# bioinfologics/w2rap-contigger

Hardware: NVIDIA B200
Metric: step-2 K=60 graph build Gbases/s (higher is better)
Workload: dtype u64

## Files before the change

### w2rap-contigger_b200/csrc/count_part.cuh

```cuda
#pragma once
#include "kernels.cuh"
#include "shard.cuh"

namespace w2r {

constexpr uint32_t MINI_TILE = 192;
constexpr uint32_t MINI_NU = 8;
constexpr uint32_t MAP_CHUNK = 512;
struct MiniParams {
    uint32_t logP, npass, pass;
    uint32_t* count;
    uint32_t* kcount;
    SkmRec* tmp;
    uint32_t* tpart;
    unsigned long long* tmp_cursor;
    uint64_t tmp_cap;
    int* overflow;
};
__global__ void __launch_bounds__(256, 6) k_minimizer_map(ReadsView r, uint64_t first, uint64_t count, const uint16_t* __restrict__ good, MiniParams mp) {
    __shared__ uint32_t wbuf[8][MINI_TILE];
    __shared__ uint32_t sbuf[8][MINI_TILE];
    uint32_t* wb = wbuf[threadIdx.x >> 5];
    uint32_t* sl = sbuf[threadIdx.x >> 5];
    const uint32_t lane = threadIdx.x & 31u;
// ... 90 lines not shown
__global__ void __launch_bounds__(256) k_scatter_records(ScatterParams sp) {
    const unsigned long long t0 = sp.range[0], t1 = sp.range[1] < sp.tmp_cap ? sp.range[1] : sp.tmp_cap, boff = *sp.batch_off;
    for (unsigned long long i = t0 + (unsigned long long)blockIdx.x * blockDim.x + threadIdx.x; i < t1; i += (unsigned long long)gridDim.x * blockDim.x) {
        const uint32_t b = __ldcs(sp.tpart + i);
        if (b == NIL) continue;
        const ulonglong2* src = reinterpret_cast<const ulonglong2*>(sp.tmp + i);
        const ulonglong2 lo = __ldcs(src), hi = __ldcs(src + 1);
        const unsigned long long pos = boff + sp.base[b] + atomicAdd(sp.cursor + b, 1u);
        if (pos < sp.recs_cap) { ulonglong2* dst = reinterpret_cast<ulonglong2*>(sp.recs + pos); dst[0] = lo; dst[1] = hi; }
        else atomicExch(sp.overflow, 1);
    }
}
__global__ void k_copy_scalar(const unsigned long long* src, unsigned long long* dst) { *dst = *src; }

__global__ void k_next_batch_off(unsigned long long* batch_off, const uint64_t* total) { batch_off[1] = batch_off[0] + *total; }

struct RegionParams {
    CountSlot* region;
    uint32_t logR;
    uint32_t sub_mask, sub_id;
    int* overflow;
};
constexpr uint32_t REGION_MAX_PROBE = 2048;
constexpr uint32_t COUNT_STOP_REGION = 1u << 24;

__device__ __forceinline__ void ld_slot(const CountSlot* q, uint64_t& w0, uint64_t& w1, uint64_t& meta) {
    uint64_t pad;
    asm volatile("ld.global.cg.v4.u64 {%0,%1,%2,%3}, [%4];" : "=l"(w0), "=l"(w1), "=l"(meta), "=l"(pad) : "l"(q));
}

__device__ __forceinline__ void region_insert(const RegionParams& rp, Kmer k, uint32_t ctx, uint64_t h) {
    const uint64_t mask = (1ull << rp.logR) - 1;
    uint64_t s = h >> (64 - rp.logR);
    for (uint32_t probe = 0; probe < REGION_MAX_PROBE; ++probe) {
        CountSlot* q = rp.region + s;
        uint64_t w0, w1, meta;
        ld_slot(q, w0, w1, meta);
        bool hit = false;
        uint32_t have = (uint32_t)(meta >> 32);
        if (w0 == k.w0 && w1 == k.w1) hit = true;
        else if (w0 == EMPTY_W0) {
            U128 old = cas128(q, ~0ull, ~0ull, k.w0, k.w1);
            hit = (old.lo == ~0ull && old.hi == ~0ull) || (old.lo == k.w0 && old.hi == k.w1);
            have = 0;
        }
        if (hit) {
            if ((uint32_t)meta < COUNT_STOP_REGION || w0 == EMPTY_W0) atomicAdd(&q->count, 1u);
            if ((have & ctx) != ctx) atomicOr(&q->ctx, ctx);
            return;
        }
        s = (s + 1) & mask;
    }
    atomicExch(rp.overflow, 1);
}

struct RunView { const uint64_t* part_base; const unsigned long long* slab_off; uint64_t P; const uint32_t* plist; };
__global__ void __launch_bounds__(256) k_count_region(const SkmRec* __restrict__ recs, const uint32_t* __restrict__ sizes, uint32_t b_first, uint32_t gy, RunView rv,
                                                      RegionParams rp) {
    const uint32_t src = blockIdx.y / gy;
    const uint32_t bi = b_first + (blockIdx.y - src * gy);
    const uint32_t b = rv.plist ? rv.plist[bi] : bi;
    const uint64_t n = sizes[(uint64_t)src * rv.P + b];
    const SkmRec* base = recs + rv.slab_off[src] + rv.part_base[(uint64_t)src * rv.P + b];
    const uint32_t lane = threadIdx.x & 31u;
    const uint64_t nw = ((uint64_t)gridDim.x * blockDim.x) >> 5;
    for (uint64_t i = ((uint64_t)blockIdx.x * blockDim.x + threadIdx.x) >> 5; i < n; i += nw) {
        const uint64_t* q = base[i].q;
        if (lane < skm_n(q[3])) {
            Kmer k; uint32_t ctx;
            skm_kmer_at(q, lane, &k, &ctx);
            const uint64_t h = kmer_hash(k);
            if (!rp.sub_mask || (((uint32_t)(h >> 3)) & rp.sub_mask) == rp.sub_id) region_insert(rp, k, ctx, h);
        }
    }
}

constexpr uint32_t SMEM_LOG_SLOTS_MAX = 13;
constexpr uint32_t SMEM_MAX_PROBE = 512;
constexpr uint32_t COUNT_STOP = 1u << 16;
constexpr uint32_t SMEM_MAX_BATCH = 16;
constexpr uint32_t SKM_CHUNK = 1024;
struct SmemCountParams {
    const SkmRec* recs;
    const uint32_t* cursor;
    const uint64_t* part_base;
    const unsigned long long* batch_off;
    uint32_t nbatch;
    uint32_t P;
    uint32_t min_freq;
    unsigned long long* hist;
    ulonglong2* solid_out; unsigned long long* solid_cursor; uint64_t solid_cap; int* solid_overflow;
    DumpRec* dump_out; unsigned long long* dump_cursor;
    uint32_t* failed; unsigned long long* failed_cursor;
    uint32_t log_slots;
    uint32_t chunk;
    const uint32_t* plist; uint32_t nlist;
};

__device__ __forceinline__ uint32_t smem_addr(const void* p) { return (uint32_t)__cvta_generic_to_shared(p); }
__device__ __forceinline__ void mbar_init(uint64_t* bar, uint32_t count) { asm volatile("mbarrier.init.shared::cta.b64 [%0], %1;" ::"r"(smem_addr(bar)), "r"(count)); }
__device__ __forceinline__ void mbar_expect_tx(uint64_t* bar, uint32_t bytes) { asm volatile("mbarrier.expect_tx.relaxed.cta.shared::cta.b64 [%0], %1;" ::"r"(smem_addr(bar)), "r"(bytes) : "memory"); }
__device__ __forceinline__ void mbar_arrive(uint64_t* bar) { asm volatile("{\n\t.reg .b64 st;\n\tmbarrier.arrive.shared::cta.b64 st, [%0];\n\t}" ::"r"(smem_addr(bar)) : "memory"); }
__device__ __forceinline__ void mbar_wait(uint64_t* bar, uint32_t parity) {
    asm volatile(
        "{\n\t.reg .pred p;\n\t"
        "WAIT_%=:\n\t"
        "mbarrier.try_wait.parity.shared::cta.b64 p, [%0], %1;\n\t"
        "@p bra DONE_%=;\n\t"
        "bra WAIT_%=;\n\t"
        "DONE_%=:\n\t}" ::"r"(smem_addr(bar)), "r"(parity) : "memory");
}
__device__ __forceinline__ void bulk_g2s(void* dst, const void* src, uint32_t bytes, uint64_t* bar) {
    asm volatile("cp.async.bulk.shared::cluster.global.mbarrier::complete_tx::bytes [%0], [%1], %2, [%3];" ::"r"(smem_addr(dst)), "l"(src), "r"(bytes), "r"(smem_addr(bar)) : "memory");
}

__device__ __forceinline__ uint32_t smem_slot_hash(Kmer k) {
    uint32_t x = (uint32_t)k.w0 * 0x9e3779b1u + (uint32_t)(k.w0 >> 32) * 0x85ebca77u;
    x ^= x >> 15;
    x += (uint32_t)(k.w1 >> 8) * 0xc2b2ae3du + (uint32_t)(k.w1 >> 40) * 0x27d4eb2fu;
    x ^= x >> 13; x *= 0x165667b1u; x ^= x >> 16;
    return x;
}

__device__ __forceinline__ U128 cas128_shared(void* addr, uint64_t cmp_lo, uint64_t cmp_hi, uint64_t val_lo, uint64_t val_hi) {
    U128 old;
    asm volatile(
        "{\n\t.reg .b128 c, v, o;\n\t"
        "mov.b128 c, {%2, %3};\n\t"
        "mov.b128 v, {%4, %5};\n\t"
        "atom.shared.relaxed.cta.cas.b128 o, [%6], c, v;\n\t"
        "mov.b128 {%0, %1}, o;\n\t}"
        : "=l"(old.lo), "=l"(old.hi)
        : "l"(cmp_lo), "l"(cmp_hi), "l"(val_lo), "l"(val_hi), "r"(smem_addr(addr))
        : "memory");
    return old;
}
__device__ __forceinline__ ulonglong2 lds128_volatile(const void* addr) {
    ulonglong2 v;
    asm volatile("ld.volatile.shared.v2.u64 {%0, %1}, [%2];" : "=l"(v.x), "=l"(v.y) : "r"(smem_addr(addr)) : "memory");
    return v;
}

__global__ void __launch_bounds__(1024, 1) k_count_smem(SmemCountParams sp) {
    extern __shared__ __align__(16) unsigned char smem_raw[];
    const uint32_t SMEM_SLOTS = 1u << sp.log_slots;
    ulonglong2* keys = reinterpret_cast<ulonglong2*>(smem_raw);
    uint32_t* ccs = reinterpret_cast<uint32_t*>(keys + SMEM_SLOTS);
    SkmRec* stage = reinterpret_cast<SkmRec*>(smem_raw + (size_t)20 * SMEM_SLOTS);
    const uint32_t CHUNK = sp.chunk;
    __shared__ __align__(8) uint64_t mbar[2];
    __shared__ unsigned int sh_hist[104];
    __shared__ int sh_fail;
    __shared__ uint32_t sh_tot[2], sh_cnt[2];
    const uint32_t lane = threadIdx.x & 31u, warp = threadIdx.x >> 5, nwarp = blockDim.x >> 5;
    const unsigned le_mask = (2u << lane) - 1u;
    for (int j = threadIdx.x; j < 104; j += blockDim.x) sh_hist[j] = 0;
    if (threadIdx.x == 0) { mbar_init(&mbar[0], 1); mbar_init(&mbar[1], 1); asm volatile("fence.mbarrier_init.release.cluster;" ::: "memory"); }
    __syncthreads();
    const uint32_t n_todo = sp.plist ? sp.nlist : sp.P;
    uint32_t cu_cnt = 0, nx_cnt = 0;
    const SkmRec* cu_src = nullptr; const SkmRec* nx_src = nullptr;
    auto load_desc = [&](uint32_t pi, uint32_t& cnt, const SkmRec*& src) {
        cnt = 0; src = nullptr;
        if (pi < n_todo && lane < sp.nbatch) {
            const uint32_t p = sp.plist ? sp.plist[pi] : pi;
            cnt = sp.cursor[(uint64_t)lane * sp.P + p];
            src = sp.recs + sp.batch_off[lane] + sp.part_base[(uint64_t)lane * sp.P + p];
        }
    };
    auto issue = [&](uint32_t cnt, const SkmRec* src, uint32_t c, uint32_t bf) {
        const uint32_t lo = c * CHUNK, hi = lo + CHUNK;
        uint32_t incl = cnt;
#pragma unroll
        for (int d = 1; d < 32; d <<= 1) { const uint32_t t = __shfl_up_sync(0xffffffffu, incl, d); if ((int)lane >= d) incl += t; }
        const uint32_t acc = incl - cnt, tot = __shfl_sync(0xffffffffu, incl, 31);
        const uint32_t s = acc > lo ? acc : lo, e = acc + cnt < hi ? acc + cnt : hi;
        if (s < e) {
            mbar_expect_tx(&mbar[bf], (e - s) * (uint32_t)sizeof(SkmRec));
            bulk_g2s(stage + (size_t)bf * CHUNK + (s - lo), src + (s - acc), (e - s) * (uint32_t)sizeof(SkmRec), &mbar[bf]);
        }
        __syncwarp();
        if (lane == 0) {
            sh_tot[bf] = tot;
            sh_cnt[bf] = (tot < hi ? tot : hi) - (tot < lo ? tot : lo);
            mbar_arrive(&mbar[bf]);
        }
    };
    uint32_t it = 0;
    if (warp == 0) {
        load_desc(blockIdx.x, cu_cnt, cu_src);
        load_desc(blockIdx.x + gridDim.x, nx_cnt, nx_src);
        if (blockIdx.x < n_todo) issue(cu_cnt, cu_src, 0, 0);
    }
    for (uint32_t pi = blockIdx.x; pi < n_todo; pi += gridDim.x) {
        const uint32_t p = sp.plist ? sp.plist[pi] : pi;
        {
            const ulonglong2 ff = make_ulonglong2(~0ull, ~0ull);
            for (uint32_t j = threadIdx.x; j < SMEM_SLOTS; j += blockDim.x) keys[j] = ff;
            uint4* cw = reinterpret_cast<uint4*>(ccs);
            for (uint32_t j = threadIdx.x; j < SMEM_SLOTS / 4; j += blockDim.x) cw[j] = make_uint4(0, 0, 0, 0);
        }
        if (threadIdx.x == 0) sh_fail = 0;
        __syncthreads();
        auto insert = [&](const Kmer k, const uint32_t ctx) {
            uint32_t s = smem_slot_hash(k) >> (32 - sp.log_slots);
            bool done = false;
            for (uint32_t probe = 0; probe < SMEM_MAX_PROBE && !done; ++probe) {
                ulonglong2 cur = lds128_volatile(keys + s);
                while (cur.x != ~0ull && cur.y == ~0ull) cur = lds128_volatile(keys + s);
                bool mine = cur.x == k.w0 && cur.y == k.w1;
                if (!mine && cur.x == ~0ull) {
                    const U128 old = cas128_shared(keys + s, ~0ull, ~0ull, k.w0, k.w1);
                    mine = (old.lo == ~0ull && old.hi == ~0ull) || (old.lo == k.w0 && old.hi == k.w1);
                }
                if (mine) {
                    const uint32_t old = atomicAdd(ccs + s, 1u);
                    if ((old & 0xffffffu) >= COUNT_STOP) atomicSub(ccs + s, 1u);
                    if ((((old >> 24) & ctx) != ctx)) atomicOr(ccs + s, ctx << 24);
                    done = true;
                } else s = (s + 1u) & (SMEM_SLOTS - 1u);
            }
            if (!done) sh_fail = 1;
        };
        for (uint32_t c = 0;; ++c, ++it) {
            const uint32_t bf = it & 1u;
            mbar_wait(&mbar[bf], (it >> 1) & 1u);
            const uint32_t tot = sh_tot[bf], cnt = sh_cnt[bf];
            const bool more = (uint64_t)(c + 1) * CHUNK < tot;
            if (warp == 0) {
                if (more) issue(cu_cnt, cu_src, c + 1, bf ^ 1u);
                else {
                    if (pi + gridDim.x < n_todo) issue(nx_cnt, nx_src, 0, bf ^ 1u);
                    cu_cnt = nx_cnt; cu_src = nx_src;
                    load_desc(pi + 2 * gridDim.x, nx_cnt, nx_src);
                }
            }
            const SkmRec* st = stage + (size_t)bf * CHUNK;
            const uint32_t share = (cnt + nwarp - 1) / nwarp;
            const uint32_t w_end = (warp + 1) * share < cnt ? (warp + 1) * share : cnt;
            for (uint32_t g0 = warp * share; g0 < w_end; g0 += 32u) {
                const uint32_t gn = w_end - g0 < 32u ? w_end - g0 : 32u;
                const bool have = lane < gn;
                const uint64_t hdr = have ? st[g0 + lane].q[3] : 0ull;
                const uint32_t nr = have ? skm_n(hdr) : 0u;
                uint32_t incl = nr;
#pragma unroll
                for (int d = 1; d < 32; d <<= 1) { const uint32_t t = __shfl_up_sync(0xffffffffu, incl, d); if ((int)lane >= d) incl += t; }
                const uint32_t total = __shfl_sync(0xffffffffu, incl, 31), excl = incl - nr;
                uint32_t before_window = 0;
                for (uint32_t t = 0; t < total; t += 32) {
                    const uint32_t rel = excl - t;
                    const unsigned starts = __reduce_or_sync(0xffffffffu, (nr && rel < 32u) ? 1u << rel : 0u);
                    const uint32_t rr = before_window + (uint32_t)__popc(starts & le_mask) - 1u;
                    const uint32_t r_excl = __shfl_sync(0xffffffffu, excl, rr & 31u);
                    const uint64_t r_hdr = __shfl_sync(0xffffffffu, hdr, rr & 31u);
                    if (t + lane < total) {
                        Kmer k; uint32_t ctx;
                        skm_kmer_at(st[g0 + rr].q, r_hdr, t + lane - r_excl, &k, &ctx);
                        insert(k, ctx);
                    }
                    before_window += (uint32_t)__popc(starts);
                }
            }
            __syncthreads();
            if (!more) { ++it; break; }
        }
        const bool failed = sh_fail != 0;
        if (failed) {
            if (threadIdx.x == 0) sp.failed[atomicAdd(sp.failed_cursor, 1ull)] = p;
        } else {
            for (uint32_t base = 0; base < SMEM_SLOTS; base += blockDim.x) {
                const uint32_t j = base + threadIdx.x;
                const bool in = j < SMEM_SLOTS;
                const ulonglong2 kk = in ? keys[j] : make_ulonglong2(~0ull, ~0ull);
                const bool occ = kk.x != ~0ull;
                const uint32_t cc = in ? ccs[j] : 0u;
                uint32_t c = cc & 0xffffffu; if (c > 255u) c = 255u;
                const uint32_t ctx = cc >> 24;
                const unsigned ones = __ballot_sync(0xffffffffu, occ && c == 1u);
                if (lane == 0 && ones) atomicAdd(&sh_hist[1], (unsigned)__popc(ones));
                if (occ && c != 1u) atomicAdd(&sh_hist[c > 100u ? 100u : c], 1u);
                const bool solid = occ && c >= sp.min_freq;
                const uint64_t pos = warp_append(sp.solid_cursor, solid);
                if (solid) { if (pos < sp.solid_cap) sp.solid_out[pos] = make_ulonglong2(kk.x, kk.y | ctx); else atomicExch(sp.solid_overflow, 1); }
                if (sp.dump_out) {
                    const uint64_t dp = warp_append(sp.dump_cursor, occ);
                    if (occ) sp.dump_out[dp] = DumpRec{kk.x, kk.y, c, ctx, NIL, 0};
                }
            }
        }
        __syncthreads();
    }
    __syncthreads();
    for (int j = threadIdx.x; j <= 100; j += blockDim.x) if (sh_hist[j]) atomicAdd(&sp.hist[j], (unsigned long long)sh_hist[j]);
}

struct ScanParams {
    CountSlot* region;
    uint64_t R;
    uint32_t min_freq;
    unsigned long long* hist;
    ulonglong2* solid_out;
    unsigned long long* solid_cursor;
    uint64_t solid_cap;
    DumpRec* dump_out;
    unsigned long long* dump_cursor;
    const int* overflow;
    int* solid_overflow;
};
__global__ void __launch_bounds__(256) k_scan_region(ScanParams sp) {
    __shared__ unsigned int sh[104];
    for (int j = threadIdx.x; j < 104; j += blockDim.x) sh[j] = 0;
    __syncthreads();
    const bool failed = *sp.overflow != 0;
    uint4* raw = reinterpret_cast<uint4*>(sp.region);
    const uint4 key_empty = make_uint4(0xffffffffu, 0xffffffffu, 0xffffffffu, 0xffffffffu), zero = make_uint4(0, 0, 0, 0);
    for (uint64_t base = (uint64_t)blockIdx.x * blockDim.x; base < sp.R; base += (uint64_t)gridDim.x * blockDim.x) {
        uint64_t i = base + threadIdx.x;
        bool occ = false, solid = false;
        uint32_t c = 0, ctx = 0;
        ulonglong2 k = make_ulonglong2(0, 0);
        if (i < sp.R) {
            k = __ldcg(reinterpret_cast<const ulonglong2*>(sp.region + i));
            if (k.x != EMPTY_W0) {
                occ = true;
                uint2 m = __ldcg(reinterpret_cast<const uint2*>(&sp.region[i].count));
                c = m.x > 255u ? 255u : m.x; ctx = m.y & 0xffu;
                raw[2 * i] = key_empty; raw[2 * i + 1] = zero;
            }
        }
        if (failed) continue;
        uint32_t bin = occ ? (c > 100u ? 100u : c) : 103u;
        unsigned peers = __match_any_sync(0xffffffffu, bin);
        if (occ && (peers & ((1u << lane_id()) - 1u)) == 0) atomicAdd(&sh[bin], (unsigned)__popc(peers));
        solid = occ && c >= sp.min_freq;
        uint64_t pos = warp_append(sp.solid_cursor, solid);
        if (solid) { if (pos < sp.solid_cap) sp.solid_out[pos] = make_ulonglong2(k.x, k.y | ctx); else atomicExch(sp.solid_overflow, 1); }
        if (sp.dump_out) {
            uint64_t dp = warp_append(sp.dump_cursor, occ);
            if (occ) sp.dump_out[dp] = DumpRec{k.x, k.y, c, ctx, NIL, 0};
        }
    }
    __syncthreads();
    if (!failed) {
        for (int j = threadIdx.x; j <= 100; j += blockDim.x) if (sh[j]) atomicAdd(&sp.hist[j], (unsigned long long)sh[j]);
    }
}

}
```

### w2rap-contigger_b200/csrc/extract.cuh

```cuda
#pragma once
#include "kmer.cuh"

namespace w2r {

struct KmerCursor {
    const uint8_t* bases;
    Kmer f, r;
    uint64_t buf;
    uint32_t j, last, prev_first;
    bool live;
    W2R_HD KmerCursor() : bases(nullptr), f{0, 0}, r{0, 0}, buf(0), j(0), last(0), prev_first(0), live(false) {}
    W2R_HD void open(const uint8_t* b, uint32_t good_len) {
        live = good_len > (uint32_t)K;
        if (!live) return;
        bases = b; f = kmer_at(b, 0); r = kmer_rc(f); last = good_len - K; j = 0; prev_first = 0; buf = 0;
    }
    W2R_HD bool next(Kmer* canon, uint32_t* ctx) {
        if (!live) return false;
        uint32_t nxt = 0, c = 0;
        if ((j & 31u) == 0) buf = bases32_at(bases, (uint64_t)j + K);
        if (j < last) { nxt = (uint32_t)buf & 3u; c |= 1u << nxt; }
        buf >>= 2;
        if (j > 0) c |= 16u << prev_first;
        const bool rev = kmer_less(r, f);
        *canon = Kmer{rev ? r.w0 : f.w0, rev ? r.w1 : f.w1};
        *ctx = rev ? ctx_rc(c) : c;
        if (j == last) live = false;
        else { prev_first = kmer_first(f); f = kmer_succ(f, nxt); r = kmer_pred(r, 3u - nxt); ++j; }
        return true;
    }
};

template <class Emit>
W2R_HD void extract_read_kmers(const uint8_t* bases, uint32_t good_len, Emit& emit) {
    KmerCursor cur;
    cur.open(bases, good_len);
    Kmer k; uint32_t ctx;
    while (cur.next(&k, &ctx)) emit(k, ctx);
}

constexpr uint32_t SKM_MAX = 32;
struct alignas(16) SkmRec { uint64_t q[4]; };
W2R_HD uint32_t skm_n(uint64_t hdr) { return (uint32_t)((hdr >> 56) & 31u) + 1u; }
W2R_HD SkmRec skm_build(const uint8_t* bases, uint32_t j_first, uint32_t n, uint32_t last) {
    const uint32_t hp = j_first > 0 ? 1u : 0u, hs = j_first + n - 1u < last ? 1u : 0u;
    const uint64_t p0 = (uint64_t)j_first - hp;
    const uint32_t bits = 2u * (n + (uint32_t)K - 1u + hp + hs);
    const uintptr_t addr = (uintptr_t)bases + (uintptr_t)(p0 >> 2);
    const uint64_t* w = (const uint64_t*)(addr & ~(uintptr_t)7);
    const uint32_t sh = (uint32_t)(addr & 7u) * 8u + (uint32_t)(p0 & 3u) * 2u;
    const uint64_t a = w[0], b = w[1], c = w[2], d = w[3];
    SkmRec r;
    r.q[0] = sh ? (a >> sh) | (b << (64u - sh)) : a;
    r.q[1] = sh ? (b >> sh) | (c << (64u - sh)) : b;
    r.q[2] = sh ? (c >> sh) | (d << (64u - sh)) : c;
    if (bits < 128u) { r.q[1] &= (1ull << (bits - 64u)) - 1ull; r.q[2] = 0; }
    else if (bits < 192u) r.q[2] = bits > 128u ? r.q[2] & ((1ull << (bits - 128u)) - 1ull) : 0ull;
    r.q[3] = ((uint64_t)(n - 1u) << 56) | ((uint64_t)hp << 61) | ((uint64_t)hs << 62);
    return r;
}
W2R_HD void skm_kmer_at(const uint64_t* q, uint64_t hdr , uint32_t j, Kmer* canon, uint32_t* ctx) {
    const uint32_t n = skm_n(hdr), hp = (uint32_t)(hdr >> 61) & 1u, hs = (uint32_t)(hdr >> 62) & 1u;
    const uint32_t b = 2u * (hp + j), wo = b >> 6, sh = b & 63u;
    const uint64_t A = q[wo], B = q[wo + 1], C = wo ? 0ull : q[2];
    const uint64_t lo = sh ? (A >> sh) | (B << (64u - sh)) : A;
    const uint64_t hi = sh ? (B >> sh) | (C << (64u - sh)) : B;
    const Kmer f{rev2(lo), rev2(hi) & ~0xffull};
    const Kmer rc{(~hi << 8) | (~lo >> 56), ~lo << 8};
    uint32_t c = 0;
    if (j + 1u < n || hs) c |= 1u << ((uint32_t)(hi >> 56) & 3u);
    if (j > 0u || hp) c |= 16u << (sh ? (uint32_t)(A >> (sh - 2u)) & 3u : (uint32_t)(q[wo - 1] >> 62));
    const bool rev = kmer_less(rc, f);
    *canon = Kmer{rev ? rc.w0 : f.w0, rev ? rc.w1 : f.w1};
    *ctx = rev ? ctx_rc(c) : c;
}
W2R_HD void skm_kmer_at(const uint64_t* q, uint32_t j, Kmer* canon, uint32_t* ctx) { skm_kmer_at(q, q[3], j, canon, ctx); }

constexpr int MINI_M = 15;
constexpr int MINI_W = K - MINI_M + 1;
W2R_HD uint32_t mmer_hash_of(uint32_t v) {
    const uint32_t rc = rev2_32(~v) >> (32 - 2 * MINI_M);
    uint32_t c = v < rc ? v : rc;
    c ^= c >> 16; c *= 0x85ebca6bu; c ^= c >> 13; c *= 0xc2b2ae35u; c ^= c >> 16;
    return c;
}
W2R_HD uint32_t mmer_hash_at(const uint8_t* bases, uint64_t pos) { return mmer_hash_of(bases16_at(bases, pos) & ((1u << (2 * MINI_M)) - 1u)); }
W2R_HD uint32_t mini_mix(uint32_t wmin) {
    uint32_t x = wmin * 0x9e3779b1u;
    x ^= x >> 15; x *= 0x2c1b3c6du; x ^= x >> 13;
    return x;
}
W2R_HD uint32_t mini_part(uint32_t mixed, uint32_t logP) { return logP ? mixed >> (32u - logP) : 0u; }
W2R_HD uint32_t kmer_minimizer_hash_words(Kmer k) {
    const uint64_t lo = rev2(k.w0), hi = rev2(k.w1);
    uint32_t m = 0xffffffffu;
    for (int t = 0; t < MINI_W; ++t) {
        const int bit = 2 * t;
        const uint64_t w = bit == 0 ? lo : (bit < 64 ? (lo >> bit) | (hi << (64 - bit)) : hi >> (bit - 64));
        const uint32_t h = mmer_hash_of((uint32_t)w & ((1u << (2 * MINI_M)) - 1u));
        if (h < m) m = h;
    }
    return m;
}
W2R_HD uint32_t kmer_minimizer_hash(const uint8_t* bases, uint64_t j) {
    uint32_t m = 0xffffffffu;
    for (int t = 0; t < MINI_W; ++t) { const uint32_t h = mmer_hash_at(bases, j + t); if (h < m) m = h; }
    return m;
}

}
```

### w2rap-contigger_b200/csrc/kernels.cuh

```cuda
#pragma once
#include "extract.cuh"
#include "kmer.cuh"
#include "path.cuh"
#include "pqvec.cuh"
#include "rt.cuh"
#include "unipath.cuh"

namespace w2r {

struct ReadsView {
    uint64_t n;
    const uint8_t* bases;
    const uint64_t* base_off;
    const uint32_t* len;
    const uint8_t* quals;
    const uint64_t* qual_off;
};

struct U128 { uint64_t lo, hi; };

__device__ __forceinline__ U128 cas128(void* addr, uint64_t cmp_lo, uint64_t cmp_hi, uint64_t val_lo, uint64_t val_hi) {
    U128 old;
    asm volatile(
        "{\n\t.reg .b128 c, v, o;\n\t"
        "mov.b128 c, {%2, %3};\n\t"
        "mov.b128 v, {%4, %5};\n\t"
        "atom.global.relaxed.gpu.cas.b128 o, [%6], c, v;\n\t"
        "mov.b128 {%0, %1}, o;\n\t}"
        : "=l"(old.lo), "=l"(old.hi)
        : "l"(cmp_lo), "l"(cmp_hi), "l"(val_lo), "l"(val_hi), "l"(addr)
        : "memory");
    return old;
}

__device__ __forceinline__ unsigned lane_id() { return threadIdx.x & 31u; }

__device__ __forceinline__ uint64_t warp_append(unsigned long long* cursor, bool want) {
    unsigned active = __activemask();
    unsigned m = __ballot_sync(active, want);
    if (!want) return 0;
    int leader = __ffs(m) - 1;
    unsigned long long base = 0;
    if ((int)lane_id() == leader) base = atomicAdd(cursor, (unsigned long long)__popc(m));
    base = __shfl_sync(m, base, leader);
    return base + __popc(m & ((1u << lane_id()) - 1u));
}
__device__ __forceinline__ void warp_add(unsigned long long* counter, unsigned long long v) {
    unsigned active = __activemask();
    for (int d = 16; d > 0; d >>= 1) v += __shfl_down_sync(active, v, d);
    if (lane_id() == 0 && v) atomicAdd(counter, v);
}


__global__ void k_init_count_table(CountSlot* tab, uint64_t T) {
    const uint4 key = make_uint4(0xffffffffu, 0xffffffffu, 0xffffffffu, 0xffffffffu), zero = make_uint4(0, 0, 0, 0);
    uint4* p = reinterpret_cast<uint4*>(tab);
    for (uint64_t i = (uint64_t)blockIdx.x * blockDim.x + threadIdx.x; i < 2 * T; i += (uint64_t)gridDim.x * blockDim.x) p[i] = (i & 1) ? zero : key;
}

__global__ void k_good_len(ReadsView r, uint64_t first, uint64_t count, uint32_t min_qual, uint16_t* __restrict__ good, unsigned long long* __restrict__ n_inst,
                           int* __restrict__ bad) {
    const uint64_t end = first + count;
    for (uint64_t base = first + (uint64_t)blockIdx.x * blockDim.x; base < end; base += (uint64_t)gridDim.x * blockDim.x) {
        uint64_t i = base + threadIdx.x;
        unsigned long long mine = 0;
        if (i < end) {
            uint32_t nq = 0;
            uint32_t gl = pq_good_length(r.quals + r.qual_off[i], r.quals + r.qual_off[i + 1], min_qual, &nq);
            if (nq != r.len[i]) atomicExch(bad, 1);
            if (gl > r.len[i]) gl = r.len[i];
            good[i] = (uint16_t)gl;
            if (gl > (uint32_t)K) mine = gl - K + 1;
        }
        unsigned active = __activemask();
        for (int d = 16; d > 0; d >>= 1) mine += __shfl_down_sync(active, mine, d);
        if (lane_id() == 0 && mine) atomicAdd(n_inst, mine);
    }
}

struct DumpRec { uint64_t w0, w1; uint32_t count, ctx, edge, off; };
__global__ void k_dump_solid(SolidTable st, DumpRec* __restrict__ out, unsigned long long* cursor) {
    const uint64_t T = st.size();
    for (uint64_t base = (uint64_t)blockIdx.x * blockDim.x; base < T; base += (uint64_t)gridDim.x * blockDim.x) {
        uint64_t i = base + threadIdx.x;
        bool want = i < T && st.slots[i].w0 != EMPTY_W0;
        uint64_t pos = warp_append(cursor, want);
        if (want) { const SolidSlot& s = st.slots[i]; out[pos] = DumpRec{s.w0, s.w1, 0, s.ctx & 0xffu, s.edge, s.off}; }
    }
}

__global__ void k_insert_solid(const ulonglong2* __restrict__ recs, uint64_t n, SolidTable st, uint32_t* __restrict__ bloom, uint32_t bloom_W, uint32_t slice_words) {
    for (uint64_t i = (uint64_t)blockIdx.x * blockDim.x + threadIdx.x; i < n; i += (uint64_t)gridDim.x * blockDim.x) {
        ulonglong2 rec = __ldcs(recs + i);
        Kmer k{rec.x, rec.y & ~0xffull};
        uint32_t ctx = (uint32_t)rec.y & 0xffu;
        if (bloom) { const uint32_t bh = bloom_hash(k); atomicOr(bloom + pd_bloom_word(bloom_W, slice_words, bh), bloom_mask(bh)); }
        uint64_t h = st.home(k);
        for (;;) {
            SolidSlot* p = st.slots + h;
            U128 old = cas128(p, ~0ull, ~0ull, k.w0, k.w1);
            if (old.lo == ~0ull && old.hi == ~0ull) { p->ctx = ctx; p->edge = NIL; p->off = 0; p->pad = 0; break; }
            h = st.next(h);
        }
    }
}
__global__ void k_insert_entries(const SolidSlot* __restrict__ recs, uint64_t n, SolidTable st, uint32_t* __restrict__ bloom, uint32_t bloom_W, uint32_t slice_words) {
    for (uint64_t i = (uint64_t)blockIdx.x * blockDim.x + threadIdx.x; i < n; i += (uint64_t)gridDim.x * blockDim.x) {
        const SolidSlot e = recs[i];
        if (bloom) { const uint32_t bh = bloom_hash(Kmer{e.w0, e.w1}); atomicOr(bloom + pd_bloom_word(bloom_W, slice_words, bh), bloom_mask(bh)); }
        uint64_t h = st.home(Kmer{e.w0, e.w1});
        for (;;) {
            SolidSlot* p = st.slots + h;
            U128 old = cas128(p, ~0ull, ~0ull, e.w0, e.w1);
            if (old.lo == ~0ull && old.hi == ~0ull) { p->ctx = e.ctx; p->edge = e.edge; p->off = e.off; p->pad = 0; break; }
            h = st.next(h);
        }
    }
}

__global__ void k_adjacency(SolidTable st) {
    const uint64_t T = st.size();
    for (uint64_t i = (uint64_t)blockIdx.x * blockDim.x + threadIdx.x; i < T; i += (uint64_t)gridDim.x * blockDim.x) {
        SolidSlot* s = st.slots + i;
        if (s->w0 == EMPTY_W0 || slot_is_ghost(*s)) continue;
        uint32_t c = s->ctx & 0xffu;
        uint32_t c2 = pruned_context(st, Kmer{s->w0, s->w1}, c);
        if (c2 != c) s->ctx = c2;
    }
}

__global__ void k_links(SolidTable st, uint32_t* __restrict__ next0, int* __restrict__ missing) {
    const uint64_t nn = 2 * st.size();
    for (uint64_t x = (uint64_t)blockIdx.x * blockDim.x + threadIdx.x; x < nn; x += (uint64_t)gridDim.x * blockDim.x) {
        int miss = 0;
        next0[x] = unipath_succ_link(st, (uint32_t)x, &miss);
        if (miss) atomicExch(missing, 1);
    }
}
__global__ void k_rank_init(const uint32_t* __restrict__ next0, uint64_t nn, RankState* __restrict__ A) {
    for (uint64_t x = (uint64_t)blockIdx.x * blockDim.x + threadIdx.x; x < nn; x += (uint64_t)gridDim.x * blockDim.x) A[x] = rank_init_node(next0, (uint32_t)x);
}
__global__ void k_rank_init_list(const uint32_t* __restrict__ list, uint64_t n, const uint32_t* __restrict__ next0, RankState* __restrict__ A) {
    for (uint64_t i = (uint64_t)blockIdx.x * blockDim.x + threadIdx.x; i < n; i += (uint64_t)gridDim.x * blockDim.x) { uint32_t x = list[i]; A[x] = rank_init_node(next0, x); }
}
__global__ void k_rank_step(const uint32_t* __restrict__ list, uint64_t n, const RankState* __restrict__ A, RankState* __restrict__ B, unsigned long long* __restrict__ unresolved) {
    for (uint64_t base = (uint64_t)blockIdx.x * blockDim.x; base < n; base += (uint64_t)gridDim.x * blockDim.x) {
        uint64_t i = base + threadIdx.x;
        bool un = false;
        if (i < n) {
            uint32_t x = list ? list[i] : (uint32_t)i;
            B[x] = rank_step_node(A, x, &un);
        }
        unsigned m = __ballot_sync(__activemask(), un);
        if (lane_id() == 0 && m) atomicAdd(unresolved, (unsigned long long)__popc(m));
    }
}
__global__ void k_rank_step_inplace(const uint32_t* __restrict__ list, uint64_t n, unsigned long long* S, unsigned long long* __restrict__ unresolved) {
    for (uint64_t base = (uint64_t)blockIdx.x * blockDim.x; base < n; base += (uint64_t)gridDim.x * blockDim.x) {
        uint64_t i = base + threadIdx.x;
        bool un = false;
        if (i < n) {
            uint32_t x = list[i];
            unsigned long long a = __ldcg(S + x);
            uint32_t ax = (uint32_t)a, ay = (uint32_t)(a >> 32);
            if (!(ay & RANK_RESOLVED)) {
                unsigned long long b = __ldcg(S + ax);
                uint32_t bx = (uint32_t)b, by = (uint32_t)(b >> 32);
                ay = (ay + (by & ~RANK_RESOLVED)) | (by & RANK_RESOLVED);
                __stcg(S + x, (unsigned long long)bx | ((unsigned long long)ay << 32));
                un = !(ay & RANK_RESOLVED);
            }
        }
        unsigned m = __ballot_sync(__activemask(), un);
        if (lane_id() == 0 && m) atomicAdd(unresolved, (unsigned long long)__popc(m));
    }
}
__global__ void k_count_splitters(const uint32_t* __restrict__ next0, const uint8_t* __restrict__ ghead, uint64_t nn, unsigned long long* __restrict__ count) {
    for (uint64_t base = (uint64_t)blockIdx.x * blockDim.x; base < nn; base += (uint64_t)gridDim.x * blockDim.x) {
        uint64_t x = base + threadIdx.x;
        const unsigned m = __ballot_sync(__activemask(), x < nn && node_is_splitter(next0, ghead, (uint32_t)x));
        if (lane_id() == 0 && m) atomicAdd(count, (unsigned long long)__popc(m));
    }
}
__global__ void k_list_splitters(const uint32_t* __restrict__ next0, const uint8_t* __restrict__ ghead, uint64_t nn, uint32_t* __restrict__ list, uint64_t list_cap,
                                 unsigned long long* cursor) {
    for (uint64_t base = (uint64_t)blockIdx.x * blockDim.x; base < nn; base += (uint64_t)gridDim.x * blockDim.x) {
        uint64_t x = base + threadIdx.x;
        bool sp = x < nn && node_is_splitter(next0, ghead, (uint32_t)x);
        uint64_t pos = warp_append(cursor, sp);
        if (sp && pos < list_cap) list[pos] = (uint32_t)x;
    }
}
__global__ void k_splitter_walk(const uint32_t* __restrict__ next0, const uint32_t* __restrict__ list, uint64_t n, RankState* __restrict__ label, RankState* __restrict__ S) {
    for (uint64_t i = (uint64_t)blockIdx.x * blockDim.x + threadIdx.x; i < n; i += (uint64_t)gridDim.x * blockDim.x) splitter_walk(next0, list[i], label, S);
}
__global__ void k_splitter_finish(const uint32_t* __restrict__ next0, uint64_t nn, RankState* __restrict__ label_then_rank, const RankState* __restrict__ S,
                                  unsigned long long* __restrict__ unresolved) {
    for (uint64_t base = (uint64_t)blockIdx.x * blockDim.x; base < nn; base += (uint64_t)gridDim.x * blockDim.x) {
        uint64_t x = base + threadIdx.x;
        bool un = false;
        if (x < nn) { RankState r = splitter_finish_node(next0, label_then_rank, S, (uint32_t)x); label_then_rank[x] = r; un = !(r.y & RANK_RESOLVED); }
        unsigned m = __ballot_sync(__activemask(), un);
        if (lane_id() == 0 && m) atomicAdd(unresolved, (unsigned long long)__popc(m));
    }
}
__global__ void k_copy_list(const uint32_t* __restrict__ list, uint64_t n, const RankState* __restrict__ src, RankState* __restrict__ dst) {
    for (uint64_t i = (uint64_t)blockIdx.x * blockDim.x + threadIdx.x; i < n; i += (uint64_t)gridDim.x * blockDim.x) dst[list[i]] = src[list[i]];
}
__global__ void k_collect_unresolved(const RankState* __restrict__ A, uint64_t nn, uint32_t* __restrict__ list, unsigned long long* cursor) {
    for (uint64_t base = (uint64_t)blockIdx.x * blockDim.x; base < nn; base += (uint64_t)gridDim.x * blockDim.x) {
        uint64_t x = base + threadIdx.x;
        bool want = x < nn && !(A[x].y & RANK_RESOLVED);
        uint64_t pos = warp_append(cursor, want);
        if (want) list[pos] = (uint32_t)x;
    }
}
__global__ void k_cycle_init(const uint32_t* __restrict__ list, uint64_t n, const uint32_t* __restrict__ next0, RankState* __restrict__ A) {
    for (uint64_t i = (uint64_t)blockIdx.x * blockDim.x + threadIdx.x; i < n; i += (uint64_t)gridDim.x * blockDim.x) {
        uint32_t x = list[i];
        A[x] = RankState{next0[x], x >> 1};
    }
}
__global__ void k_cycle_step(const uint32_t* __restrict__ list, uint64_t n, SolidTable st, const RankState* __restrict__ A, RankState* __restrict__ B, int* __restrict__ changed) {
    for (uint64_t i = (uint64_t)blockIdx.x * blockDim.x + threadIdx.x; i < n; i += (uint64_t)gridDim.x * blockDim.x) {
        uint32_t x = list[i];
        bool ch;
        B[x] = cycle_step_node(st, A, x, &ch);
        if (ch) *changed = 1;
    }
}
__global__ void k_cycle_cut(const uint32_t* __restrict__ list, uint64_t n, const RankState* __restrict__ A, uint32_t* __restrict__ next0) {
    for (uint64_t i = (uint64_t)blockIdx.x * blockDim.x + threadIdx.x; i < n; i += (uint64_t)gridDim.x * blockDim.x) {
        cycle_cut_node(A, next0, list[i]);
    }
}
__global__ void k_strand_decide(SolidTable st, const RankState* __restrict__ R, uint8_t* __restrict__ keep, int* __restrict__ too_long) {
    const uint64_t nn = 2 * st.size();
    for (uint64_t xi = (uint64_t)blockIdx.x * blockDim.x + threadIdx.x; xi < nn; xi += (uint64_t)gridDim.x * blockDim.x) {
        if (strand_decide_node(st, R, (uint32_t)xi, keep)) atomicExch(too_long, 1);
    }
}
__global__ void k_collect_heads(SolidTable st, const RankState* __restrict__ R, const uint8_t* __restrict__ keep, uint32_t* __restrict__ h_node,
                                uint64_t* __restrict__ h_w0, uint64_t* __restrict__ h_w1, uint32_t* __restrict__ h_n, unsigned long long* cursor, uint64_t cap) {
    const uint64_t nn = 2 * st.size();
    for (uint64_t base = (uint64_t)blockIdx.x * blockDim.x; base < nn; base += (uint64_t)gridDim.x * blockDim.x) {
        uint64_t xi = base + threadIdx.x;
        bool want = false;
        uint32_t x = (uint32_t)xi;
        if (xi < nn) want = head_is_kept(st, R, keep, x);
        uint64_t pos = warp_append(cursor, want);
        if (want && pos < cap) {
            Kmer k = node_kmer(st, x);
            h_node[pos] = x; h_w0[pos] = k.w0; h_w1[pos] = k.w1; h_n[pos] = (R[x].y & ~RANK_RESOLVED) + 1u;
        }
    }
}
__global__ void k_assign_edges(const uint32_t* __restrict__ perm, uint64_t E, const uint32_t* __restrict__ h_node, const uint32_t* __restrict__ h_n,
                               uint32_t* __restrict__ edge_of_head, uint32_t* __restrict__ edge_len, uint32_t* __restrict__ edge_nbytes) {
    for (uint64_t i = (uint64_t)blockIdx.x * blockDim.x + threadIdx.x; i < E; i += (uint64_t)gridDim.x * blockDim.x) {
        uint32_t j = perm[i];
        edge_of_head[h_node[j]] = (uint32_t)i;
        uint32_t len = h_n[j] + K - 1;
        edge_len[i] = len;
        edge_nbytes[i] = (len + 3) / 4;
    }
}
struct OrBase {
    uint8_t* bases;
    __device__ __forceinline__ void operator()(uint64_t byte_off, uint64_t pos, uint32_t b) const {
        uint64_t addr = byte_off + (pos >> 2);
        atomicOr(reinterpret_cast<uint32_t*>(bases + (addr & ~3ull)), b << (8 * (uint32_t)(addr & 3ull) + 2 * (uint32_t)(pos & 3ull)));
    }
};
__global__ void k_emit_edges(SolidTable st, const RankState* __restrict__ R, const uint32_t* __restrict__ edge_of_head, const uint64_t* __restrict__ edge_off,
                             uint8_t* __restrict__ edge_bases) {
    const uint64_t nn = 2 * st.size();
    OrBase put{edge_bases};
    for (uint64_t xi = (uint64_t)blockIdx.x * blockDim.x + threadIdx.x; xi < nn; xi += (uint64_t)gridDim.x * blockDim.x) emit_node(st, R, edge_of_head, edge_off, (uint32_t)xi, put);
}

__global__ void k_copy_to_host(const uint8_t* __restrict__ src, uint8_t* __restrict__ dst, size_t bytes) {
    const size_t n16 = bytes / 16;
    const uint4* s4 = reinterpret_cast<const uint4*>(src);
    uint4* d4 = reinterpret_cast<uint4*>(dst);
    for (size_t i = (size_t)blockIdx.x * blockDim.x + threadIdx.x; i < n16; i += (size_t)gridDim.x * blockDim.x) d4[i] = s4[i];
    if (blockIdx.x == 0 && threadIdx.x < (bytes & 15)) dst[n16 * 16 + threadIdx.x] = src[n16 * 16 + threadIdx.x];
}

__global__ void k_edge_ends(const uint8_t* __restrict__ edge_bases, const uint64_t* __restrict__ edge_off, const uint32_t* __restrict__ edge_len, uint64_t E,
                            uint64_t* __restrict__ kh, uint64_t* __restrict__ k0, uint64_t* __restrict__ k1, uint8_t* __restrict__ is_pal) {
    for (uint64_t idx = (uint64_t)blockIdx.x * blockDim.x + threadIdx.x; idx < 4 * E; idx += (uint64_t)gridDim.x * blockDim.x) {
        uint64_t e = idx >> 2;
        uint32_t w = (uint32_t)idx & 3u;
        bool pal; EndKey key;
        edge_end_key(edge_bases + edge_off[e], edge_len[e], w, &pal, &key);
        if (w == 0) is_pal[e] = pal ? 1 : 0;
        kh[idx] = key.h; k0[idx] = key.k0; k1[idx] = key.k1;
    }
}
__global__ void k_vertex_flags(const uint32_t* __restrict__ perm, uint64_t n4, const uint64_t* __restrict__ kh, const uint64_t* __restrict__ k0,
                               const uint64_t* __restrict__ k1, uint32_t* __restrict__ flag) {
    for (uint64_t i = (uint64_t)blockIdx.x * blockDim.x + threadIdx.x; i < n4; i += (uint64_t)gridDim.x * blockDim.x) {
        uint32_t j = perm[i];
        bool valid = !(kh[j] == ~0ull && k0[j] == ~0ull && k1[j] == ~0ull);
        uint32_t fl = 0;
        if (valid) {
            if (i == 0) fl = 1;
            else { uint32_t q = perm[i - 1]; fl = (kh[q] != kh[j] || k0[q] != k0[j] || k1[q] != k1[j]) ? 1u : 0u; }
        }
        flag[i] = fl;
    }
}
__global__ void k_hash_order_check(const uint32_t* __restrict__ perm, uint64_t n4, const uint64_t* __restrict__ kh, const uint64_t* __restrict__ k0,
                                   const uint64_t* __restrict__ k1, unsigned long long* __restrict__ collisions) {
    for (uint64_t i = (uint64_t)blockIdx.x * blockDim.x + threadIdx.x + 1; i < n4; i += (uint64_t)gridDim.x * blockDim.x) {
        const uint32_t j = perm[i], q = perm[i - 1];
        if (kh[q] == kh[j] && (k0[q] != k0[j] || k1[q] != k1[j])) atomicAdd(collisions, 1ull);
    }
}
__global__ void k_scatter_vids(const uint32_t* __restrict__ perm, uint64_t n4, const uint32_t* __restrict__ flag, const uint32_t* __restrict__ excl,
                               const uint64_t* __restrict__ kh, const uint64_t* __restrict__ k0, const uint64_t* __restrict__ k1, int32_t* __restrict__ edge_vertices) {
    for (uint64_t i = (uint64_t)blockIdx.x * blockDim.x + threadIdx.x; i < n4; i += (uint64_t)gridDim.x * blockDim.x) {
        uint32_t j = perm[i];
        bool valid = !(kh[j] == ~0ull && k0[j] == ~0ull && k1[j] == ~0ull);
        edge_vertices[j] = valid ? (int32_t)(excl[i] + flag[i]) - 1 : -1;
    }
}
__global__ void k_pal_widths(const uint8_t* __restrict__ is_pal, uint64_t E, uint32_t* __restrict__ width) {
    for (uint64_t i = (uint64_t)blockIdx.x * blockDim.x + threadIdx.x; i < E; i += (uint64_t)gridDim.x * blockDim.x) width[i] = is_pal[i] ? 1u : 2u;
}
__global__ void k_hbv_edges(uint64_t E, const uint8_t* __restrict__ is_pal, const uint32_t* __restrict__ xl, const int32_t* __restrict__ edge_vertices,
                            int32_t* __restrict__ fwd_xlat, int32_t* __restrict__ rev_xlat, uint32_t* __restrict__ hcanon, int32_t* __restrict__ hleft, int32_t* __restrict__ hright,
                            int32_t* __restrict__ involution) {
    for (uint64_t i = (uint64_t)blockIdx.x * blockDim.x + threadIdx.x; i < E; i += (uint64_t)gridDim.x * blockDim.x) {
        uint32_t f = xl[i];
        fwd_xlat[i] = (int32_t)f;
        hcanon[f] = (uint32_t)(i << 1); hleft[f] = edge_vertices[4 * i]; hright[f] = edge_vertices[4 * i + 1];
        if (is_pal[i]) { rev_xlat[i] = (int32_t)f; involution[f] = (int32_t)f; }
        else {
            rev_xlat[i] = (int32_t)f + 1; hcanon[f + 1] = (uint32_t)(i << 1) | 1u; hleft[f + 1] = edge_vertices[4 * i + 2]; hright[f + 1] = edge_vertices[4 * i + 3];
            involution[f] = (int32_t)f + 1; involution[f + 1] = (int32_t)f;
        }
    }
}
__global__ void k_adj_fill(uint64_t nh, const int32_t* __restrict__ hleft, const int32_t* __restrict__ hright, int32_t* __restrict__ from_e, int32_t* __restrict__ to_e,
                           uint32_t* __restrict__ from_cnt, uint32_t* __restrict__ to_cnt, int* __restrict__ bad) {
    for (uint64_t he = (uint64_t)blockIdx.x * blockDim.x + threadIdx.x; he < nh; he += (uint64_t)gridDim.x * blockDim.x) {
        int32_t l = hleft[he], r = hright[he];
        uint32_t a = atomicAdd(&from_cnt[l], 1u);
        if (a < 4) from_e[4 * (int64_t)l + a] = (int32_t)he; else atomicExch(bad, 1);
        uint32_t b = atomicAdd(&to_cnt[r], 1u);
        if (b < 4) to_e[4 * (int64_t)r + b] = (int32_t)he; else atomicExch(bad, 1);
    }
}
__global__ void k_adj_sort(uint64_t nv, const int32_t* __restrict__ hleft, const int32_t* __restrict__ hright, int32_t* __restrict__ from_e, int32_t* __restrict__ to_e,
                           const uint32_t* __restrict__ from_cnt, const uint32_t* __restrict__ to_cnt, uint8_t* __restrict__ from_n, uint8_t* __restrict__ to_n) {
    for (uint64_t v = (uint64_t)blockIdx.x * blockDim.x + threadIdx.x; v < nv; v += (uint64_t)gridDim.x * blockDim.x) {
        for (int dir = 0; dir < 2; ++dir) {
            int32_t* lst = (dir ? to_e : from_e) + 4 * v;
            const int32_t* nb = dir ? hleft : hright;
            uint32_t n = dir ? to_cnt[v] : from_cnt[v];
            if (n > 4) n = 4;
            for (uint32_t i = 1; i < n; ++i) {
                int32_t e = lst[i]; int32_t ke = nb[e];
                int j = (int)i - 1;
                while (j >= 0 && (nb[lst[j]] > ke || (nb[lst[j]] == ke && lst[j] > e))) { lst[j + 1] = lst[j]; --j; }
                lst[j + 1] = e;
            }
            (dir ? to_n : from_n)[v] = (uint8_t)n;
        }
    }
}

struct alignas(8) PathMeta { uint32_t x, y; };
constexpr int PATH_GAP_BATCH = 4;
template <int MIN_CTAS>
__global__ void __launch_bounds__(128, MIN_CTAS) k_path_reads(ReadsView r, GraphView g, const uint32_t* __restrict__ list, uint64_t n_rows,
                                                    int32_t* __restrict__ stage, uint32_t cap, uint32_t left_cap, int32_t* __restrict__ out_offset,
                                                    PathMeta* __restrict__ out_meta, uint32_t apply_fixpaths) {
    struct Slot { PathState st; uint32_t pad[(sizeof(PathState) / 4) % 2 == 0 ? 1 : 2]; };
    __shared__ Slot slots[128];
    PathState& ps = slots[threadIdx.x].st;
    const uint32_t lane = lane_id();
    const uint64_t stride = (uint64_t)gridDim.x * blockDim.x;
    for (uint64_t row0 = (uint64_t)blockIdx.x * blockDim.x + (threadIdx.x & ~31u); row0 < n_rows; row0 += stride) {
        const uint64_t row = row0 + lane;
        const bool live = row < n_rows;
        const uint64_t i = live ? (list ? list[row] : row) : 0;
        PathWalker w(ps);
        w.init(g, r.bases + r.base_off[i], live ? r.len[i] : 0u, stage + (live ? row : 0) * cap, cap, left_cap);
        bool need = false, run = true, have_gap = false;
        uint32_t from = 0, found_p = 0;
        const SolidSlot* found_slot = nullptr;
        for (;;) {
            if (run) {
                if (have_gap) w.gap_found(found_p, found_slot);
                need = w.scan();
                from = ps.itr + 1u;
                run = false; have_gap = false;
            }
            unsigned m = __ballot_sync(0xffffffffu, need);
            if (!m) break;
            uint32_t cand = 0;
            while (m) {
                int src[PATH_GAP_BATCH];
                uint32_t word[PATH_GAP_BATCH], bits[PATH_GAP_BATCH];
                int n = 0;
#pragma unroll
                for (int q = 0; q < PATH_GAP_BATCH; ++q) { src[q] = m ? __ffs((int)m) - 1 : -1; if (m) { m &= m - 1; ++n; } }
#pragma unroll
                for (int q = 0; q < PATH_GAP_BATCH; ++q) {
                    word[q] = 0; bits[q] = 1;
                    if (q < n) {
                        const uint8_t* b = reinterpret_cast<const uint8_t*>(__shfl_sync(0xffffffffu, reinterpret_cast<unsigned long long>(ps.bases), src[q]));
                        const uint32_t p = __shfl_sync(0xffffffffu, from, src[q]) + lane, nk = __shfl_sync(0xffffffffu, ps.nk, src[q]);
                        if (p < nk) {
                            Kmer f, rc;
                            kmer_pair_at(b, p, &f, &rc);
                            const uint32_t hh = bloom_hash(kmer_less(rc, f) ? rc : f);
                            if (g.dict.bloom) { word[q] = __ldg(g.dict.bloom + pd_bloom_word(g.dict.W, g.dict.slice_words, hh)); bits[q] = bloom_mask(hh); }
                            else { word[q] = 1; bits[q] = 1; }
                        }
                    }
                }
#pragma unroll
                for (int q = 0; q < PATH_GAP_BATCH; ++q) {
                    if (q < n) {
                        const unsigned mm = __ballot_sync(0xffffffffu, (word[q] & bits[q]) == bits[q]);
                        if ((int)lane == src[q]) cand = mm;
                    }
                }
// ... 93 lines not shown
```

### w2rap-contigger_b200/csrc/pipeline.cu

```cuda
#include <algorithm>
#include <cmath>
#include <chrono>
#include <cstdarg>
#include <exception>
#include <map>
#include <mutex>
#include <thread>
#include <unordered_map>

#include <cuda.h>

#include "../../include/w2rap_step2.h"
#include "device_reads.cuh"
#include "count_part.cuh"
#include "kernels.cuh"
#include "shardgraph_kernels.cuh"
#include "nccl_dl.h"
#include "prims.cuh"
#include "slab_freelist.h"
#include "places.cuh"

namespace w2r {

static double now_ms() { return std::chrono::duration<double, std::milli>(std::chrono::steady_clock::now().time_since_epoch()).count(); }
// ... 131 lines not shown
                    CUmemAccessDesc acc = {};
                    acc.location = prop.location; acc.flags = CU_MEM_ACCESS_FLAGS_PROT_READWRITE;
                    if (v.Map(base + mapped, take, 0, h, 0) == CUDA_SUCCESS && v.SetAccess(base + mapped, take, &acc, 1) == CUDA_SUCCESS) {
                        v.Release(h);
                        fl.add_free(mapped, take);
                        mapped += take;
                        return true;
                    }
                    v.Release(h);
                    return false;
                }
            }
            cudaMemPool_t pool;
            if (attempt == 0 && cudaDeviceGetDefaultMemPool(&pool, device) == cudaSuccess) { cudaDeviceSynchronize(); cudaMemPoolTrimTo(pool, 0); } else break;
        }
        return false;
    }
    void* acquire(size_t bytes) {
        bytes = (bytes + ALIGN - 1) / ALIGN * ALIGN;
        size_t off = fl.take(bytes);
        if (off == SlabFreeList::NONE) {
            if (!grow(bytes - fl.free_tail(mapped))) return nullptr;
            off = fl.take(bytes);
            if (off == SlabFreeList::NONE) return nullptr;
        }
        return (void*)(base + off);
    }
    void release(void* p) { fl.give_back((size_t)((CUdeviceptr)p - base)); }
};
struct SlabLease {
    DeviceSlab* slab = nullptr;
    explicit SlabLease(int device) {
        DeviceSlab& s = DeviceSlab::get(device);
        if (s.lease.try_lock()) { if (s.init(device)) slab = &s; else s.lease.unlock(); }
    }
    ~SlabLease() {
        if (!slab) return;
        if (std::uncaught_exceptions() > 0) cudaDeviceSynchronize();
        slab->lease.unlock();
    }
    SlabLease(const SlabLease&) = delete;
    SlabLease& operator=(const SlabLease&) = delete;
};

template <class T>
struct SBuf {
    T* p = nullptr;
    size_t n = 0;
    cudaStream_t s = nullptr;
    DeviceSlab* slab = nullptr;
    SBuf() {}
    SBuf(Ctx& c, size_t n_) { alloc(c, n_); }
    SBuf(const SBuf&) = delete;
    SBuf& operator=(const SBuf&) = delete;
    SBuf(SBuf&& o) noexcept : p(o.p), n(o.n), s(o.s), slab(o.slab) { o.p = nullptr; o.n = 0; o.slab = nullptr; }
    SBuf& operator=(SBuf&& o) noexcept { if (this != &o) { release(); p = o.p; n = o.n; s = o.s; slab = o.slab; o.p = nullptr; o.n = 0; o.slab = nullptr; } return *this; }
    ~SBuf() { release(); }
    void alloc(Ctx& c, size_t n_) {
        release();
        s = c.stream; n = n_;
        if (!n) return;
        const double t0 = now_ms();
        const size_t bytes = n * sizeof(T);
        DeviceSlab* sl = (DeviceSlab*)c.slab;
        if (sl && bytes >= DeviceSlab::MIN_BYTES) { p = (T*)sl->acquire(bytes); if (p) slab = sl; }
        cudaError_t e = cudaSuccess;
        if (!p) e = cudaMallocAsync((void**)&p, bytes, s);
        const double dt = now_ms() - t0;
        g_alloc_host_ms += dt;
        if (dt > 20.0 && getenv("W2RAP_TRACE")) fprintf(stderr, "[w2rap] device allocation of %.2f GB took %.1f ms on the host\n", bytes / 1e9, dt);
        W2R_CUDA(e);
    }
    void release() {
        if (p) {
            const double t0 = now_ms();
            if (slab) slab->release(p); else cudaFreeAsync(p, s);
            g_alloc_host_ms += now_ms() - t0;
        }
        p = nullptr; n = 0; slab = nullptr;
    }
    size_t bytes() const { return n * sizeof(T); }
    void zero() { if (n) W2R_CUDA(cudaMemsetAsync(p, 0, bytes(), s)); }
    void fill_ff() { if (n) W2R_CUDA(cudaMemsetAsync(p, 0xff, bytes(), s)); }
};

static size_t device_budget(const Ctx& c) {
    size_t fr = 0, tot = 0;
    W2R_CUDA(cudaMemGetInfo(&fr, &tot));
    cudaMemPool_t pool;
    if (cudaDeviceGetDefaultMemPool(&pool, c.device) == cudaSuccess) {
        uint64_t reserved = 0, used = 0;
        cudaMemPoolGetAttribute(pool, cudaMemPoolAttrReservedMemCurrent, &reserved);
        cudaMemPoolGetAttribute(pool, cudaMemPoolAttrUsedMemCurrent, &used);
        if (reserved > used) fr += (size_t)(reserved - used);
    }
    if (c.slab) fr += ((const DeviceSlab*)c.slab)->idle_bytes();
    return fr;
}

struct StageTimer {
    Ctx& c;
    cudaEvent_t ev[2];
    explicit StageTimer(Ctx& c_) : c(c_) { cudaEventCreate(&ev[0]); cudaEventCreate(&ev[1]); }
    ~StageTimer() { cudaEventDestroy(ev[0]); cudaEventDestroy(ev[1]); }
    void start() { cudaEventRecord(ev[0], c.stream); }
    float stop() { cudaEventRecord(ev[1], c.stream); cudaEventSynchronize(ev[1]); float ms = 0; cudaEventElapsedTime(&ms, ev[0], ev[1]); return ms; }
};

struct KernelTimers {
    struct Span { int idx; cudaEvent_t a, b; };
    std::vector<Span> spans;
    cudaStream_t s = nullptr;
    void begin(int idx) { Span sp{idx, nullptr, nullptr}; cudaEventCreate(&sp.a); cudaEventCreate(&sp.b); cudaEventRecord(sp.a, s); spans.push_back(sp); }
    void end() { cudaEventRecord(spans.back().b, s); }
    void resolve(float* kernel_ms) {
        for (Span& sp : spans) {
            float ms = 0;
            if (cudaEventSynchronize(sp.b) == cudaSuccess && cudaEventElapsedTime(&ms, sp.a, sp.b) == cudaSuccess) kernel_ms[sp.idx] += ms; else cudaGetLastError();
            cudaEventDestroy(sp.a); cudaEventDestroy(sp.b);
        }
        spans.clear();
    }
    ~KernelTimers() { for (Span& sp : spans) { cudaEventDestroy(sp.a); cudaEventDestroy(sp.b); } }
};
#define W2R_TIMED(idx, ...) do { kt_.begin(idx); __VA_ARGS__; kt_.end(); } while (0)

static void say(const Ctx& c, const char* fmt, ...) {
    if (!c.verbose) return;
    va_list ap; va_start(ap, fmt); vprintf(fmt, ap); va_end(ap); printf("\n"); fflush(stdout);
}

struct Pipeline {
    Ctx c;
    const DeviceReads& dr;
    const w2rap_params& prm;
    w2rap_graph* out;
    GraphOwner* owner;
    std::vector<DumpRec> dump_host;
    KernelTimers kt_;

    double trace_t0 = 0;
    void trace_mark(const char* what) {
        static const bool on = getenv("W2RAP_TRACE") != nullptr;
        if (!on) return;
        cudaStreamSynchronize(c.stream);
        const double t = now_ms();
        if (trace_t0 && rank == 0) fprintf(stderr, "[w2rap] %-28s %8.1f ms   (allocator so far %.1f ms)\n", what, t - trace_t0, g_alloc_host_ms);
        trace_t0 = t;
    }

    SBuf<uint16_t> good;
    SBuf<SolidSlot> solid_slots;
    SolidTable st{nullptr, 0};
    uint64_t E = 0, nv = 0, nh = 0;
    SBuf<uint8_t> edge_bases; SBuf<uint64_t> edge_off; SBuf<uint32_t> edge_len;
    SBuf<int32_t> edge_vertices, fwd_xlat, rev_xlat, involution, hleft, hright, from_e, to_e;
    SBuf<uint32_t> hcanon;
    SBuf<uint8_t> from_n, to_n;
    uint64_t edge_bytes = 0;
    int world = 1, rank = 0;
    ncclComm_t comm = nullptr;

    Pipeline(const DeviceReads& dr_, const w2rap_params& p_, w2rap_graph* out_, GraphOwner* ow) : dr(dr_), prm(p_), out(out_), owner(ow) {}

    unsigned grid(uint64_t n, unsigned block, unsigned per_sm = 16) const { return grid_for(c, n, block, per_sm); }

    void set_l2_window(void* base, size_t bytes) {
        cudaStreamAttrValue attr;
        memset(&attr, 0, sizeof attr);
        attr.accessPolicyWindow.base_ptr = base;
        attr.accessPolicyWindow.num_bytes = bytes;
        attr.accessPolicyWindow.hitRatio = 1.0f;
        attr.accessPolicyWindow.hitProp = bytes ? cudaAccessPropertyPersisting : cudaAccessPropertyNormal;
        attr.accessPolicyWindow.missProp = bytes ? cudaAccessPropertyStreaming : cudaAccessPropertyNormal;
        if (cudaStreamSetAttribute(c.stream, cudaStreamAttributeAccessPolicyWindow, &attr) != cudaSuccess) cudaGetLastError();
    }

    void nccl_check(ncclResult_t r, const char* what) {
        if (r != ncclSuccess) W2R_FAIL(W2RAP_ERR_CUDA, "NCCL %s failed: %s", what, NcclApi::get().GetErrorString ? NcclApi::get().GetErrorString(r) : "?");
    }
    void allreduce_u64(std::vector<unsigned long long>& v, ncclRedOp_t op) {
        if (world == 1) return;
        SBuf<unsigned long long> d(c, v.size());
        W2R_CUDA(cudaMemcpyAsync(d.p, v.data(), v.size() * 8, cudaMemcpyHostToDevice, c.stream));
        nccl_check(NcclApi::get().AllReduce(d.p, d.p, v.size(), ncclUint64, op, comm, c.stream), "all-reduce");
        W2R_CUDA(cudaMemcpyAsync(v.data(), d.p, v.size() * 8, cudaMemcpyDeviceToHost, c.stream));
        W2R_CUDA(cudaStreamSynchronize(c.stream));
    }
    void alltoall_slabs(const void* send, void* recv, size_t slab_bytes) {
        NcclApi& n = NcclApi::get();
        nccl_check(n.GroupStart(), "group start");
        for (int peer = 0; peer < world; ++peer) {
            if (peer == rank) continue;
            nccl_check(n.Send((const char*)send + (size_t)peer * slab_bytes, slab_bytes, ncclUint8, peer, comm, c.stream), "send");
            nccl_check(n.Recv((char*)recv + (size_t)peer * slab_bytes, slab_bytes, ncclUint8, peer, comm, c.stream), "recv");
        }
        nccl_check(n.GroupEnd(), "group end");
        W2R_CUDA(cudaMemcpyAsync((char*)recv + (size_t)rank * slab_bytes, (const char*)send + (size_t)rank * slab_bytes, slab_bytes, cudaMemcpyDeviceToDevice, c.stream));
    }

    void alltoall_v(const void* send, const std::vector<size_t>& soff, const std::vector<size_t>& scnt, void* recv, const std::vector<size_t>& roff,
                    const std::vector<size_t>& rcnt) {
        NcclApi& n = NcclApi::get();
        nccl_check(n.GroupStart(), "group start");
        for (int peer = 0; peer < world; ++peer) {
            if (peer == rank) continue;
            if (scnt[peer]) nccl_check(n.Send((const char*)send + soff[peer], scnt[peer], ncclUint8, peer, comm, c.stream), "send");
            if (rcnt[peer]) nccl_check(n.Recv((char*)recv + roff[peer], rcnt[peer], ncclUint8, peer, comm, c.stream), "recv");
        }
        nccl_check(n.GroupEnd(), "group end");
        if (scnt[rank]) W2R_CUDA(cudaMemcpyAsync((char*)recv + roff[rank], (const char*)send + soff[rank], scnt[rank], cudaMemcpyDeviceToDevice, c.stream));
    }

    struct Batch { uint64_t first, count; cudaEvent_t ready; };
    struct CountPlan {
        uint32_t logP = 0, npass = 1, nmap = 1, nslab = 1;
        uint64_t P = 1, Pown = 1;
        uint64_t n_inst = 0, n_inst_local = 0;
    };
    struct CountBufs {
        SBuf<SkmRec> recs, xrecs;
        SBuf<SkmRec> tmp; SBuf<uint32_t> tpart;
        SBuf<unsigned long long> tmp_cursor, tmp_range;
        SBuf<uint32_t> part_count, part_kcount, cursor;
        SBuf<uint64_t> part_base, batch_total, batch_ktotal;
        SBuf<unsigned long long> batch_off;
        SBuf<uint32_t> xcount, xkcount;
        SBuf<uint64_t> xbase, xtot, xktot;
        SBuf<unsigned long long> xoff;
    };
    SBuf<unsigned long long> cs_scal;
    SBuf<int> cs_flags;
    SBuf<unsigned long long> cs_hist;
    SBuf<CountSlot> cs_region;
    SBuf<DumpRec> cs_dump;
    SBuf<ulonglong2> cs_solid; uint64_t cs_solid_cap = 0;
    uint64_t cs_R = 0; uint32_t cs_logR = 0;
    bool good_done = false;
    float map_ms = 0, reduce_ms = 0, xchg_ms = 0;
    uint32_t n_groups = 0;
    uint64_t xchg_bytes = 0, xchg_count_bytes = 0, n_records = 0;

    void run_good_len(const Batch& bt) {
        if (bt.ready) W2R_CUDA(cudaStreamWaitEvent(c.stream, bt.ready, 0));
        if (bt.count) W2R_TIMED(W2RAP_KT_GOOD_LEN, W2R_LAUNCH(c, k_good_len, grid(bt.count, 128), 128, 0, dr.view(), bt.first, bt.count, prm.min_qual, good.p, cs_scal.p, cs_flags.p));
    }

    static unsigned map_ctas() {
        static const unsigned n = getenv("W2RAP_MAP_CTAS") ? (unsigned)atoi(getenv("W2RAP_MAP_CTAS")) : 6u;
        return n;
    }
    uint64_t map_chunk_warps(uint64_t count) const { return std::min<uint64_t>(count, (uint64_t)grid(count * 32, 256, map_ctas()) * 8); }

    bool map_records(const CountPlan& pl, CountBufs& cb, const std::vector<Batch>& batches, uint32_t pass, uint64_t* need) {
        const ReadsView rv = dr.view();
        const uint64_t P = pl.P;
        cb.cursor.zero(); cb.part_count.zero(); cb.part_kcount.zero();
        W2R_CUDA(cudaMemsetAsync(cb.batch_off.p, 0, sizeof(unsigned long long), c.stream));
        std::vector<Batch> mb = batches;
        if (world > 1) {
            if (!good_done) for (const Batch& bt : batches) run_good_len(bt);
            good_done = true;
            mb.assign(1, Batch{0, dr.n, nullptr});
        }
        std::vector<cudaEvent_t> ev(2 * pl.nmap, nullptr);
        struct EvGuard { std::vector<cudaEvent_t>& v; ~EvGuard() { for (cudaEvent_t e : v) if (e) cudaEventDestroy(e); } } evg{ev};
        W2R_CUDA(cudaMemsetAsync(cb.tmp_cursor.p, 0, 8, c.stream));
        W2R_CUDA(cudaMemsetAsync(cb.tpart.p, 0xff, cb.tpart.bytes(), c.stream));
        for (uint32_t bi = 0; bi < pl.nmap; ++bi) {
            const Batch& bt = mb[bi];
            MiniParams mp{pl.logP, pl.npass, pass, cb.part_count.p + bi * P, cb.part_kcount.p + bi * P, cb.tmp.p, cb.tpart.p, cb.tmp_cursor.p, cb.tmp.n, cs_flags.p + 1};
            ScatterParams sp{cb.tmp.p, cb.tpart.p, cb.tmp_range.p + bi, cb.part_base.p + bi * P, cb.cursor.p + bi * P, cb.recs.p, cb.batch_off.p + bi, cb.recs.n, cb.tmp.n, cs_flags.p + 1};
            if (!good_done) run_good_len(bt);
            W2R_CUDA(cudaEventCreate(&ev[2 * bi])); W2R_CUDA(cudaEventCreate(&ev[2 * bi + 1]));
            W2R_CUDA(cudaEventRecord(ev[2 * bi], c.stream));
            W2R_LAUNCH(c, k_copy_scalar, 1, 1, 0, (const unsigned long long*)cb.tmp_cursor.p, cb.tmp_range.p + bi);
            if (bt.count && pl.n_inst_local) W2R_TIMED(W2RAP_KT_MAP, W2R_LAUNCH(c, k_minimizer_map, grid(bt.count * 32, 256, map_ctas()), 256, 0, rv, bt.first, bt.count, good.p, mp));
            W2R_LAUNCH(c, k_copy_scalar, 1, 1, 0, (const unsigned long long*)cb.tmp_cursor.p, cb.tmp_range.p + bi + 1);
            exclusive_scan<uint32_t, uint64_t>(c, cb.part_count.p + bi * P, P, cb.part_base.p + bi * P, cb.batch_total.p + bi);
            W2R_LAUNCH(c, k_next_batch_off, 1, 1, 0, cb.batch_off.p + bi, cb.batch_total.p + bi);
            if (bt.count && pl.n_inst_local) { W2R_TIMED(W2RAP_KT_SCATTER, W2R_LAUNCH(c, k_scatter_records, (unsigned)(c.sm_count * 8), 256, 0, sp)); c.count_launches++; }
            W2R_CUDA(cudaEventRecord(ev[2 * bi + 1], c.stream));
        }
        good_done = true;
        unsigned long long total = 0, staged = 0;
        W2R_CUDA(cudaMemcpyAsync(&total, cb.batch_off.p + pl.nmap, 8, cudaMemcpyDeviceToHost, c.stream));
        W2R_CUDA(cudaMemcpyAsync(&staged, cb.tmp_cursor.p, 8, cudaMemcpyDeviceToHost, c.stream));
        W2R_CUDA(cudaStreamSynchronize(c.stream));
        for (uint32_t bi = 0; bi < pl.nmap; ++bi) { float ms = 0; cudaEventElapsedTime(&ms, ev[2 * bi], ev[2 * bi + 1]); map_ms += ms; }
        if (d2h_scalar(c, cs_flags.p)) W2R_FAIL(W2RAP_ERR_BAD_ARG, "a read's quality vector does not have one quality per base");
        n_records += total;
        *need = std::max(total, staged);
        std::vector<unsigned long long> of = {(unsigned long long)d2h_scalar(c, cs_flags.p + 1)};
        allreduce_u64(of, ncclMax);
        if (of[0]) { W2R_CUDA(cudaMemsetAsync(cs_flags.p + 1, 0, sizeof(int), c.stream)); return false; }
        return true;
    }

    void exchange_records(const CountPlan& pl, CountBufs& cb) {
        EventTimer kt(c.stream);
        kt.start();
        const uint64_t Pown = pl.Pown;
        alltoall_slabs(cb.part_count.p, cb.xcount.p, Pown * sizeof(uint32_t));
        alltoall_slabs(cb.part_kcount.p, cb.xkcount.p, Pown * sizeof(uint32_t));
        W2R_CUDA(cudaMemsetAsync(cb.xoff.p, 0, sizeof(unsigned long long), c.stream));
        for (int sidx = 0; sidx < world; ++sidx) {
// ... 169 lines not shown
        cs_dump.alloc(c, prm.dump_kmers == 2 ? pl.n_inst : 0);
        W2R_LAUNCH(c, k_init_count_table, grid(4 * cs_R, 256), 256, 0, cs_region.p, 2 * cs_R);
        cudaStream_t s2 = nullptr;
        W2R_CUDA(cudaStreamCreateWithFlags(&s2, cudaStreamNonBlocking));
        struct StreamGuard { cudaStream_t s; ~StreamGuard() { if (s) { cudaStreamSynchronize(s); cudaStreamDestroy(s); } } } s2_guard{s2};
        cudaEvent_t ev_fork, ev_join;
        cudaEventCreateWithFlags(&ev_fork, cudaEventDisableTiming); cudaEventCreateWithFlags(&ev_join, cudaEventDisableTiming);
        struct EventGuard { cudaEvent_t a, b; ~EventGuard() { cudaEventDestroy(a); cudaEventDestroy(b); } } ev_guard{ev_fork, ev_join};

        std::vector<unsigned long long> rk = {dr.n_kreads};
        allreduce_u64(rk, ncclSum);
        double rec_per_inst = pl.n_inst ? std::min(1.0, 1.15 * ((double)rk[0] + 0.074 * (double)pl.n_inst) / (double)pl.n_inst) : 1.0;
        uint64_t need_exact = 0;
        pl.npass = prm.force_passes ? prm.force_passes : 1u;
        for (int attempt = 0;; ++attempt) {
            if (attempt > 12) W2R_FAIL(W2RAP_ERR_INTERNAL, "k-mer partitioning did not converge");
            const uint64_t P = pl.P, Pown = pl.Pown;
            const size_t local_recs = std::max<uint64_t>(need_exact + need_exact / 64, (uint64_t)((double)pl.n_inst_local * rec_per_inst / pl.npass * (pl.npass > 1 ? 1.25 : 1.0))) + 1024;
            const size_t solid_est = (size_t)((double)pl.n_inst / world / pl.npass / std::max<uint32_t>(1, prm.min_freq) * 1.3) * sizeof(ulonglong2);
            const size_t rec_bytes = (local_recs * 2 + local_recs / 8 + (world > 1 ? (size_t)((double)pl.n_inst * rec_per_inst / world / pl.npass * 1.25) : 0)) * (sizeof(SkmRec) + 4);
            std::vector<unsigned long long> too_big = {(rec_bytes + solid_est + cs_dump.bytes() + (64u << 20) > budget) ? 1ull : 0ull};
            allreduce_u64(too_big, ncclMax);
            if (too_big[0] && !prm.force_passes) {
                if (pl.npass >= 4096) W2R_FAIL(W2RAP_ERR_OOM, "not enough device memory for the k-mer records even in 4096 passes");
                pl.npass *= 2; --attempt; continue;
            }
            CountBufs cb;
            uint64_t chunk_warps = 0;
            if (world > 1) chunk_warps = map_chunk_warps(dr.n);
            else for (const Batch& bt : batches) chunk_warps += map_chunk_warps(bt.count);
            const size_t stage_recs = local_recs + local_recs / 8 + chunk_warps * MAP_CHUNK;
            cb.tmp_cursor.alloc(c, 1); cb.tmp_range.alloc(c, pl.nmap + 1);
            cb.part_count.alloc(c, pl.nmap * P); cb.part_kcount.alloc(c, pl.nmap * P); cb.cursor.alloc(c, pl.nmap * P);
            cb.part_base.alloc(c, pl.nmap * P); cb.batch_total.alloc(c, pl.nmap); cb.batch_ktotal.alloc(c, pl.nmap);
            cb.batch_off.alloc(c, pl.nmap + 1);
            if (world > 1) {
                cb.xcount.alloc(c, world * Pown); cb.xkcount.alloc(c, world * Pown); cb.xbase.alloc(c, world * Pown);
                cb.xtot.alloc(c, world); cb.xktot.alloc(c, world); cb.xoff.alloc(c, world + 1);
            }
            bool retry = false;
            W2R_CUDA(cudaMemsetAsync(cs_scal.p + 1, 0, 16, c.stream));
            cs_hist.zero();
            n_groups = 0;
            uint64_t solid_used = 0;
            for (uint32_t pass = 0; pass < pl.npass && !retry; ++pass) {
                uint64_t need = 0;
                cb.recs.alloc(c, local_recs);
                cb.tmp.alloc(c, stage_recs); cb.tpart.alloc(c, stage_recs);
                trace_mark("count: buffers");
                const bool mapped = map_records(pl, cb, batches, pass, &need);
                trace_mark("count: map+scatter");
                cb.tmp.release(); cb.tpart.release();
                if (!mapped) {
                    std::vector<unsigned long long> nd = {need};
                    allreduce_u64(nd, ncclMax);
                    need_exact = std::max<uint64_t>(need_exact, nd[0]);
                    retry = true; break;
                }
                if (world > 1) { exchange_records(pl, cb); cb.recs.release(); }
                trace_mark("count: exchange");
                const uint32_t* xcur = world > 1 ? cb.xcount.p : cb.part_count.p;
                const uint32_t* xkcur = world > 1 ? cb.xkcount.p : cb.part_kcount.p;
                const SkmRec* xrecs = world > 1 ? cb.xrecs.p : cb.recs.p;
                RunView runs = world > 1 ? RunView{cb.xbase.p, cb.xoff.p, Pown, nullptr} : RunView{cb.part_base.p, cb.batch_off.p, Pown, nullptr};
                {
                    SBuf<uint64_t> ktot(c, pl.nslab), kscan(c, Pown);
                    for (uint32_t sidx = 0; sidx < pl.nslab; ++sidx) exclusive_scan<uint32_t, uint64_t>(c, xkcur + (uint64_t)sidx * Pown, Pown, kscan.p, ktot.p + sidx);
                    std::vector<uint64_t> kt_h(pl.nslab);
                    W2R_CUDA(cudaMemcpyAsync(kt_h.data(), ktot.p, pl.nslab * 8, cudaMemcpyDeviceToHost, c.stream));
                    W2R_CUDA(cudaStreamSynchronize(c.stream));
                    uint64_t owned = 0;
                    for (uint64_t v : kt_h) owned += v;
                    const uint64_t want = solid_used + owned / std::max<uint32_t>(1, prm.min_freq) + 1024;
                    if (want > cs_solid_cap) {
                        SBuf<ulonglong2> bigger(c, want + want / 4);
                        if (solid_used) W2R_CUDA(cudaMemcpyAsync(bigger.p, cs_solid.p, solid_used * sizeof(ulonglong2), cudaMemcpyDeviceToDevice, c.stream));
                        cs_solid = std::move(bigger);
                        cs_solid_cap = cs_solid.n;
                    }
                }
                trace_mark("count: solid staging");
                reduce_records(pl, xrecs, xcur, xkcur, runs, s2, ev_fork, ev_join);
                trace_mark("count: reduce");
                solid_used = d2h_scalar(c, cs_scal.p + 1);
                if (world > 1) cb.xrecs.release();
            }
            if (retry) continue;
            if (d2h_scalar(c, cs_flags.p + 2)) W2R_FAIL(W2RAP_ERR_INTERNAL, "solid staging buffer overflow");
            break;
        }
        {
            std::vector<unsigned long long> exact = {(unsigned long long)d2h_scalar(c, cs_scal.p)};
            allreduce_u64(exact, ncclSum);
            out->n_kmer_instances = exact[0];
            say(c, "%llu k-mer instances in quality-floored reads", exact[0]);
        }
        out->timings.count_kernel_ms = map_ms;
        out->timings.region_ms = reduce_ms;
        out->timings.exchange_ms = xchg_ms;
        out->timings.count_passes = n_groups;
        std::vector<unsigned long long> hh(104);
        W2R_CUDA(cudaMemcpyAsync(hh.data(), cs_hist.p, 104 * 8, cudaMemcpyDeviceToHost, c.stream));
        unsigned long long cursors[2];
        W2R_CUDA(cudaMemcpyAsync(cursors, cs_scal.p + 1, 16, cudaMemcpyDeviceToHost, c.stream));
        W2R_CUDA(cudaStreamSynchronize(c.stream));
        allreduce_u64(hh, ncclSum);
        uint64_t n_distinct = 0;
        for (int i = 1; i <= 100; ++i) { out->hist[i] = hh[i]; n_distinct += hh[i]; }
        const uint64_t n_solid_local = cursors[0];
        if (prm.dump_kmers == 2 && cursors[1]) {
            dump_host.resize(cursors[1]);
            W2R_CUDA(cudaMemcpyAsync(dump_host.data(), cs_dump.p, cursors[1] * sizeof(DumpRec), cudaMemcpyDeviceToHost, c.stream));
            W2R_CUDA(cudaStreamSynchronize(c.stream));
        }
        cs_region.release(); cs_dump.release();
        build_dictionary(n_solid_local, n_distinct);
    }

    void alloc_path_filter(uint64_t n_solid) {
        path_slice_words = 0;
        path_bloom.release();
        if (n_solid < 4096 || getenv("W2RAP_NO_BLOOM") || !prm.want_paths) return;
        static const uint64_t bloom_mb = getenv("W2RAP_BLOOM_MB") ? (uint64_t)atoi(getenv("W2RAP_BLOOM_MB")) : 192;
        const uint64_t cap = std::max<uint64_t>(bloom_mb << 20, std::min<uint64_t>(n_solid + n_solid / 2, 8ull << 30));
        uint64_t bytes = std::min<uint64_t>(cap, std::max<uint64_t>(4096, n_solid * 2));
        static const uint64_t exact_mb = getenv("W2RAP_BLOOM_EXACT_MB") ? (uint64_t)atoi(getenv("W2RAP_BLOOM_EXACT_MB")) : 0;
        if (exact_mb) bytes = exact_mb << 20;
        path_slice_words = (uint32_t)std::max<uint64_t>(64, bytes / 4 / world);
        path_bloom.alloc(c, (size_t)path_slice_words * world);
        path_bloom.zero();
    }

    uint64_t n_solid_local_ = 0;
    uint32_t count_logP_ = 0;
    SBuf<PathSlice> path_slices;
    SBuf<uint32_t> path_bloom;
    uint32_t path_slice_words = 0;
    uint64_t n_slice_entries = 0;
    cudaStream_t dict_stream = nullptr;
    cudaEvent_t dict_ready = nullptr;
    bool dict_pending = false;
    void wait_for_dictionary() { if (dict_pending) { W2R_CUDA(cudaStreamWaitEvent(c.stream, dict_ready, 0)); dict_pending = false; } }
    void build_dictionary(uint64_t n_solid_local, uint64_t n_distinct) {
        std::vector<unsigned long long> tot = {n_solid_local};
        allreduce_u64(tot, ncclSum);
        const uint64_t n_solid = tot[0];
        n_solid_local_ = n_solid_local;
        out->n_distinct = n_distinct; out->n_solid = n_solid;
        say(c, "%llu kmers counted, filtering...", (unsigned long long)n_distinct);
        say(c, "%llu / %llu kmers with Freq >= %u", (unsigned long long)n_solid, (unsigned long long)n_distinct, prm.min_freq);
        if (world > 1) return;
        EventTimer kt(c.stream);
        kt.start();
        const uint64_t nslots = solid_table_slots(n_solid);
        if (nslots > (1ull << 31) - 8) W2R_FAIL(W2RAP_ERR_OOM, "too many solid k-mers for one device's graph stage (32-bit oriented node ids); shard over more GPUs");
        solid_slots.alloc(c, nslots);
        solid_slots.fill_ff();
        st = SolidTable{solid_slots.p, nslots};
        alloc_path_filter(n_solid);
        if (n_solid) W2R_TIMED(W2RAP_KT_INSERT_SOLID, W2R_LAUNCH(c, k_insert_solid, grid(n_solid, 256), 256, 0, (const ulonglong2*)cs_solid.p, n_solid, st,
                                                                   path_slice_words ? path_bloom.p : nullptr, 1u, path_slice_words));
        out->timings.dict_ms = kt.stop();
        cs_solid.release();
    }

    void list_ranking(SBuf<uint32_t>& next0, const uint8_t* ghead, uint64_t nn, SBuf<RankState>& A, SBuf<RankState>& B, RankState** cur_out, RankState** oth_out) {
        SBuf<int> flags(c, 4); flags.zero();
        SBuf<unsigned long long> scal(c, 4); scal.zero();
        W2R_LAUNCH(c, k_count_splitters, grid(nn, 256), 256, 0, next0.p, ghead, nn, scal.p + 3);
        const uint64_t nsp = d2h_scalar(c, scal.p + 3);
        SBuf<uint32_t> splist(c, nsp);
        W2R_CUDA(cudaMemsetAsync(A.p, 0xff, A.bytes(), c.stream));
        W2R_CUDA(cudaMemsetAsync(scal.p + 3, 0, 8, c.stream));
        W2R_LAUNCH(c, k_list_splitters, grid(nn, 256), 256, 0, next0.p, ghead, nn, splist.p, nsp, scal.p + 3);
        if (nsp) W2R_TIMED(W2RAP_KT_SPLITTER_WALK, W2R_LAUNCH(c, k_splitter_walk, grid(nsp, 256), 256, 0, (const uint32_t*)next0.p, (const uint32_t*)splist.p, nsp, A.p, B.p));
        unsigned long long prev_un = ~0ull;
        if (nsp) {
            for (int round = 0; round < 48; ++round) {
                W2R_CUDA(cudaMemsetAsync(scal.p, 0, 8, c.stream));
                W2R_LAUNCH(c, k_rank_step_inplace, grid(nsp, 256), 256, 0, (const uint32_t*)splist.p, nsp, (unsigned long long*)B.p, scal.p);
                unsigned long long un = d2h_scalar(c, scal.p);
                if (un == 0 || un == prev_un) { prev_un = un; break; }
                prev_un = un;
            }
        }
        W2R_CUDA(cudaMemsetAsync(scal.p, 0, 8, c.stream));
        W2R_TIMED(W2RAP_KT_SPLITTER_FINISH, W2R_LAUNCH(c, k_splitter_finish, grid(nn, 256), 256, 0, next0.p, nn, A.p, (const RankState*)B.p, scal.p));
        prev_un = d2h_scalar(c, scal.p);
        RankState* cur = A.p; RankState* oth = B.p;
        if (prev_un) {
            uint64_t ncyc = prev_un;
            SBuf<uint32_t> list(c, ncyc);
            splist.release();
            W2R_CUDA(cudaMemsetAsync(scal.p + 1, 0, 8, c.stream));
            W2R_LAUNCH(c, k_collect_unresolved, grid(nn, 256), 256, 0, cur, nn, list.p, scal.p + 1);
            if (d2h_scalar(c, scal.p + 1) != ncyc) W2R_FAIL(W2RAP_ERR_INTERNAL, "unresolved node count changed between kernels");
            SBuf<RankState> D(c, nn);
            RankState* x0 = oth; RankState* x1 = D.p;
            W2R_LAUNCH(c, k_cycle_init, grid(ncyc, 256), 256, 0, list.p, ncyc, next0.p, x0);
            for (int round = 0; round < 40; ++round) {
                W2R_CUDA(cudaMemsetAsync(flags.p + 1, 0, sizeof(int), c.stream));
                W2R_LAUNCH(c, k_cycle_step, grid(ncyc, 256), 256, 0, list.p, ncyc, st, x0, x1, flags.p + 1);
                std::swap(x0, x1);
                if (!d2h_scalar(c, flags.p + 1)) break;
            }
            W2R_LAUNCH(c, k_cycle_cut, grid(ncyc, 256), 256, 0, list.p, ncyc, x0, next0.p);
            W2R_LAUNCH(c, k_rank_init_list, grid(ncyc, 256), 256, 0, list.p, ncyc, next0.p, x0);
            for (int round = 0; round < 40; ++round) {
                W2R_CUDA(cudaMemsetAsync(scal.p, 0, 8, c.stream));
                W2R_LAUNCH(c, k_rank_step, grid(ncyc, 256), 256, 0, list.p, ncyc, x0, x1, scal.p);
                std::swap(x0, x1);
                unsigned long long un = d2h_scalar(c, scal.p);
                if (un == 0) break;
                if (round == 39) W2R_FAIL(W2RAP_ERR_INTERNAL, "circle ranking did not converge");
            }
            W2R_LAUNCH(c, k_copy_list, grid(ncyc, 256), 256, 0, list.p, ncyc, x0, cur);
            W2R_CUDA(cudaStreamSynchronize(c.stream));
        }
        *cur_out = cur; *oth_out = oth;
    }

    void edges_from_heads(SBuf<uint32_t>& h_idx, SBuf<uint32_t>& h_n, SBuf<uint64_t>& h_w0, SBuf<uint64_t>& h_w1, SBuf<uint32_t>& edge_of) {
        SBuf<uint32_t> perm(c, E), tmp(c, E);
        if (E) {
            W2R_LAUNCH(c, k_rs_iota, grid(E, 256), 256, 0, perm.p, (uint32_t)E);
            SortWord words[2] = {{h_w1.p, 8, 64}, {h_w0.p, 0, 64}};
            radix_sort_perm(c, perm.p, tmp.p, (uint32_t)E, words, 2);
        }
        edge_len.alloc(c, E);
        SBuf<uint32_t> nbytes(c, E);
        if (E) W2R_LAUNCH(c, k_assign_edges, grid(E, 256), 256, 0, perm.p, E, h_idx.p, h_n.p, edge_of.p, edge_len.p, nbytes.p);
        edge_off.alloc(c, E + 1);
        SBuf<unsigned long long> tot(c, 1);
        exclusive_scan<uint32_t, unsigned long long>(c, nbytes.p, E, (unsigned long long*)edge_off.p, tot.p);
        edge_bytes = E ? d2h_scalar(c, tot.p) : 0;
        W2R_CUDA(cudaMemcpyAsync(edge_off.p + E, &edge_bytes, 8, cudaMemcpyHostToDevice, c.stream));
        W2R_CUDA(cudaStreamSynchronize(c.stream));
        edge_bases.alloc(c, (edge_bytes + 3 + 32) & ~3ull);
        edge_bases.zero();
    }

    void unipath_stage() {
        const uint64_t T = st.size(), nn = 2 * T;
        SBuf<uint32_t> next0(c, nn);
        SBuf<int> flags(c, 4); flags.zero();
        SBuf<unsigned long long> scal(c, 4); scal.zero();
        W2R_TIMED(W2RAP_KT_LINKS, W2R_LAUNCH(c, k_links, grid(nn, 256), 256, 0, st, next0.p, flags.p));
        if (d2h_scalar(c, flags.p)) W2R_FAIL(W2RAP_ERR_INTERNAL, "a neighbour k-mer promised by a pruned context is missing (reference: ForceAssert in EdgeBuilder::lookup)");
        SBuf<RankState> A(c, nn), B(c, nn);
        RankState* cur = nullptr; RankState* oth = nullptr;
        list_ranking(next0, nullptr, nn, A, B, &cur, &oth);
        const RankState* R = cur;
        SBuf<uint8_t> keep(c, nn); keep.zero();
        W2R_LAUNCH(c, k_strand_decide, grid(nn, 256), 256, 0, st, R, keep.p, flags.p + 2);
        if (d2h_scalar(c, flags.p + 2)) W2R_FAIL(W2RAP_ERR_EDGE_TOO_LONG, "an edge is longer than 2^24 k-mers (reference: KDef offset is 24 bits)");
        uint64_t cap = out->n_solid;
        SBuf<uint32_t> h_node(c, cap), h_n(c, cap);
        SBuf<uint64_t> h_w0(c, cap), h_w1(c, cap);
        W2R_CUDA(cudaMemsetAsync(scal.p + 2, 0, 8, c.stream));
        W2R_LAUNCH(c, k_collect_heads, grid(nn, 256), 256, 0, st, R, keep.p, h_node.p, h_w0.p, h_w1.p, h_n.p, scal.p + 2, cap);
        E = d2h_scalar(c, scal.p + 2);
        if (E > cap) W2R_FAIL(W2RAP_ERR_INTERNAL, "more edges than solid k-mers");
        SBuf<uint32_t> edge_of_head(c, nn); edge_of_head.fill_ff();
        edges_from_heads(h_node, h_n, h_w0, h_w1, edge_of_head);
        W2R_TIMED(W2RAP_KT_EMIT_EDGES, W2R_LAUNCH(c, k_emit_edges, grid(nn, 256), 256, 0, st, R, edge_of_head.p, edge_off.p, edge_bases.p));
        W2R_CUDA(cudaStreamSynchronize(c.stream));
    }

    template <class T>
    void allgather_v(const T* mine, uint64_t n_mine, SBuf<T>& all, std::vector<uint64_t>& off) {
        std::vector<unsigned long long> per(world, 0ull);
        per[rank] = n_mine;
        allreduce_u64(per, ncclSum);
        off.assign(world + 1, 0);
        for (int r = 0; r < world; ++r) off[r + 1] = off[r] + per[r];
        all.alloc(c, off[world] + 1);
        NcclApi& n = NcclApi::get();
        nccl_check(n.GroupStart(), "group start");
        for (int r = 0; r < world; ++r)
            if (per[r]) nccl_check(n.Broadcast(r == rank ? (const void*)mine : (const void*)(all.p + off[r]), all.p + off[r], per[r] * sizeof(T), ncclUint8, r, comm, c.stream), "broadcast");
        nccl_check(n.GroupEnd(), "group end");
        xchg_bytes += n_mine * sizeof(T) * (uint64_t)(world - 1);
    }

    void graph_stage_sharded(SBuf<ulonglong2>& solid, uint64_t n_local, uint32_t logP) {
        EventTimer xt(c.stream);
        float xms = 0;
        const uint32_t me = (uint32_t)rank, W = (uint32_t)world;
        SBuf<int> flags(c, 8); flags.zero();
        SBuf<unsigned long long> scal(c, 8); scal.zero();
        trace_mark("(before graph stage)");
        kt_.begin(W2RAP_KT_SG_QUERIES);
        uint64_t qcap = std::max<uint64_t>(1024, n_local / 4);
        SBuf<ulonglong2> qkeys;
        SBuf<unsigned long long> qcount(c, W);
        SBuf<uint64_t> qbase(c, W);
        std::vector<unsigned long long> qn(W, 0);
        for (int attempt = 0;; ++attempt) {
            if (attempt > 2) W2R_FAIL(W2RAP_ERR_INTERNAL, "neighbour query buffers did not converge");
            qkeys.alloc(c, W * qcap);
            std::vector<uint64_t> qb(W);
            for (uint32_t d = 0; d < W; ++d) qb[d] = d * qcap;
            W2R_CUDA(cudaMemcpyAsync(qbase.p, qb.data(), W * 8, cudaMemcpyHostToDevice, c.stream));
            qcount.zero();
            if (n_local) W2R_LAUNCH(c, k_neighbour_queries, grid(n_local, 256), 256, 0, solid.p, n_local, logP, W, me, QueryOut{qkeys.p, qbase.p, qcount.p, qcap});
            W2R_CUDA(cudaMemcpyAsync(qn.data(), qcount.p, W * 8, cudaMemcpyDeviceToHost, c.stream));
            W2R_CUDA(cudaStreamSynchronize(c.stream));
            unsigned long long mx = 0;
            for (auto v : qn) mx = std::max(mx, v);
            if (mx <= qcap) break;
            qcap = mx + mx / 32 + 64;
        }
        uint64_t nq_total = 0;
        for (auto v : qn) nq_total += v;
        kt_.end();
        trace_mark("graph: queries");
        const uint64_t nslots = solid_table_slots(n_local + nq_total);
        if (nslots > (1ull << 31) - 8) W2R_FAIL(W2RAP_ERR_OOM, "too many solid k-mers per GPU for 32-bit oriented node ids; shard over more GPUs");
        solid_slots.alloc(c, nslots);
        solid_slots.fill_ff();
        st = SolidTable{solid_slots.p, nslots};
        if (n_local) W2R_TIMED(W2RAP_KT_INSERT_SOLID, W2R_LAUNCH(c, k_insert_solid, grid(n_local, 256), 256, 0, (const ulonglong2*)solid.p, n_local, st, (uint32_t*)nullptr, 1u, 0u));
        solid.release();
        trace_mark("graph: local table");
        kt_.begin(W2RAP_KT_SG_QUERIES);
        xt.start();
        SBuf<unsigned long long> rcount(c, W);
        alltoall_slabs(qcount.p, rcount.p, sizeof(unsigned long long));
        std::vector<unsigned long long> rn(W, 0);
        W2R_CUDA(cudaMemcpyAsync(rn.data(), rcount.p, W * 8, cudaMemcpyDeviceToHost, c.stream));
        W2R_CUDA(cudaStreamSynchronize(c.stream));
        std::vector<size_t> q_off(W), q_cnt(W), r_off(W), r_cnt(W);
        uint64_t nr_total = 0;
        for (uint32_t d = 0; d < W; ++d) { q_off[d] = d * qcap; q_cnt[d] = qn[d]; r_off[d] = nr_total; r_cnt[d] = rn[d]; nr_total += rn[d]; if (d != me) xchg_bytes += qn[d] * 16 + rn[d] * 8; }
        auto scaled = [](const std::vector<size_t>& v, size_t k) { std::vector<size_t> o(v.size()); for (size_t i = 0; i < v.size(); ++i) o[i] = v[i] * k; return o; };
        SBuf<ulonglong2> rkeys(c, nr_total + 1);
        alltoall_v(qkeys.p, scaled(q_off, 16), scaled(q_cnt, 16), rkeys.p, scaled(r_off, 16), scaled(r_cnt, 16));
        SBuf<uint32_t> rreply(c, nr_total + 1), qreply(c, W * qcap), gslot(c, W * qcap);
        if (nr_total) W2R_LAUNCH(c, k_answer_queries, grid(nr_total, 256), 256, 0, st, (const ulonglong2*)rkeys.p, nr_total, rreply.p);
        alltoall_v(rreply.p, scaled(r_off, 4), scaled(r_cnt, 4), qreply.p, scaled(q_off, 4), scaled(q_cnt, 4));
        xms += xt.stop();
        rkeys.release();
        for (uint32_t d = 0; d < W; ++d)
            if (qn[d]) W2R_LAUNCH(c, k_insert_ghosts, grid(qn[d], 256), 256, 0, st, (const ulonglong2*)qkeys.p + d * qcap, (const uint32_t*)qreply.p + d * qcap, (uint64_t)qn[d], d, gslot.p + d * qcap);
        qkeys.release();
        kt_.end();
        trace_mark("graph: ghosts");
        W2R_TIMED(W2RAP_KT_ADJACENCY, W2R_LAUNCH(c, k_adjacency, grid(st.size(), 256), 256, 0, st));
        kt_.begin(W2RAP_KT_SG_QUERIES);
        xt.start();
        SBuf<uint32_t> rctx(c, nr_total + 1), qctx(c, W * qcap);
        if (nr_total) W2R_LAUNCH(c, k_gather_ctx, grid(nr_total, 256), 256, 0, st, (const uint32_t*)rreply.p, nr_total, rctx.p);
        alltoall_v(rctx.p, scaled(r_off, 4), scaled(r_cnt, 4), qctx.p, scaled(q_off, 4), scaled(q_cnt, 4));
        xms += xt.stop();
        for (uint32_t d = 0; d < W; ++d)
            if (qn[d]) W2R_LAUNCH(c, k_apply_ghost_ctx, grid(qn[d], 256), 256, 0, st, (const uint32_t*)gslot.p + d * qcap, (const uint32_t*)qctx.p + d * qcap, (uint64_t)qn[d]);
        kt_.end();
        rreply.release(); qreply.release(); gslot.release(); rctx.release(); qctx.release();
        trace_mark("graph: adjacency");
        const uint64_t nn = 2 * st.size();
        SBuf<uint32_t> next0(c, nn);
        SBuf<uint8_t> ghead(c, nn); ghead.zero();
        W2R_TIMED(W2RAP_KT_LINKS, W2R_LAUNCH(c, k_links_sharded, grid(nn, 256), 256, 0, st, next0.p, ghead.p, flags.p));
        if (d2h_scalar(c, flags.p)) W2R_FAIL(W2RAP_ERR_INTERNAL, "a neighbour k-mer promised by a pruned context is missing (reference: ForceAssert in EdgeBuilder::lookup)");
        SBuf<RankState> A(c, nn), B(c, nn);
        RankState* cur = nullptr; RankState* oth = nullptr;
        SBuf<PieceRec> pieces;
        SBuf<uint32_t> nxt, flip;
        SBuf<RankState> S;
        uint64_t np = 0, npl_last = 0;
        uint32_t piece0 = 0;
        uint32_t* lpiece = nullptr;
        for (int iteration = 0;; ++iteration) {
            if (iteration > 1) W2R_FAIL(W2RAP_ERR_INTERNAL, "circles left after cutting them");
            list_ranking(next0, ghead.p, nn, A, B, &cur, &oth);
            trace_mark("graph: links+list ranking");
            kt_.begin(W2RAP_KT_SG_PIECES);
            lpiece = reinterpret_cast<uint32_t*>(oth);
            uint32_t* lhead = lpiece + nn;
            W2R_CUDA(cudaMemsetAsync(scal.p, 0, 8, c.stream));
            W2R_LAUNCH(c, k_count_piece_heads, grid(nn, 256), 256, 0, next0.p, (const uint8_t*)ghead.p, nn, scal.p);
            const uint64_t npl = d2h_scalar(c, scal.p);
            SBuf<PieceRec> lp(c, npl);
            W2R_CUDA(cudaMemsetAsync(scal.p, 0, 8, c.stream));
            W2R_LAUNCH(c, k_emit_pieces, grid(nn, 256), 256, 0, st, (const uint32_t*)next0.p, (const uint8_t*)ghead.p, (const RankState*)cur, me, lp.p, npl, scal.p, lpiece, lhead);
            if (npl) W2R_LAUNCH(c, k_piece_flips, grid(npl, 256), 256, 0, lp.p, npl, (const uint32_t*)lhead);
            xt.start();
            std::vector<uint64_t> poff;
            allgather_v(lp.p, npl, pieces, poff);
            xms += xt.stop();
            np = poff[W]; piece0 = (uint32_t)poff[me]; npl_last = npl;
            trace_mark("graph: pieces gathered");
            if (np >= (1ull << 32) - 8) W2R_FAIL(W2RAP_ERR_OOM, "more than 2^32 chain pieces");
            lp.release();
            uint64_t msz = 64;
            while (msz < 2 * np) msz <<= 1;
            SBuf<uint64_t> mkeys(c, msz); mkeys.fill_ff();
            SBuf<uint32_t> mvals(c, msz);
            GidMap gm{mkeys.p, mvals.p, msz - 1};
            nxt.alloc(c, np); flip.alloc(c, np); S.alloc(c, np);
            SBuf<uint64_t> poff_dev(c, W + 1);
            W2R_CUDA(cudaMemcpyAsync(poff_dev.p, poff.data(), (W + 1) * 8, cudaMemcpyHostToDevice, c.stream));
            if (np) {
                W2R_LAUNCH(c, k_gidmap_insert, grid(np, 256), 256, 0, (const PieceRec*)pieces.p, np, gm);
                W2R_LAUNCH(c, k_piece_link, grid(np, 256), 256, 0, (const PieceRec*)pieces.p, np, gm, (const uint64_t*)poff_dev.p, nxt.p, flip.p, flags.p + 1);
                W2R_LAUNCH(c, k_piece_rank_init, grid(np, 256), 256, 0, (const PieceRec*)pieces.p, (const uint32_t*)nxt.p, np, S.p);
            }
            if (d2h_scalar(c, flags.p + 1)) W2R_FAIL(W2RAP_ERR_INTERNAL, "a chain piece points at a node that heads no piece");
            unsigned long long un = 0, prev = ~0ull;
            for (int round = 0; round < 64 && np; ++round) {
                for (int sub = 0; sub < 3; ++sub) {
                    W2R_CUDA(cudaMemsetAsync(scal.p, 0, 8, c.stream));
                    W2R_LAUNCH(c, k_piece_rank_step, grid(np, 256), 256, 0, (unsigned long long*)S.p, np, scal.p);
                }
                un = d2h_scalar(c, scal.p);
                if (un == 0 || un == prev) break;
                prev = un;
            }
            kt_.end();
            if (un == 0) break;
            std::vector<uint32_t> nxt_h(np);
            std::vector<RankState> S_h(np);
            W2R_CUDA(cudaMemcpyAsync(nxt_h.data(), nxt.p, np * 4, cudaMemcpyDeviceToHost, c.stream));
            W2R_CUDA(cudaMemcpyAsync(S_h.data(), S.p, np * 8, cudaMemcpyDeviceToHost, c.stream));
            W2R_CUDA(cudaMemsetAsync(scal.p, 0, 8, c.stream));
            W2R_LAUNCH(c, k_collect_cycle_nodes, grid(nn, 256), 256, 0, st, (const uint32_t*)next0.p, (const RankState*)cur, (const uint32_t*)lpiece, piece0, (const RankState*)S.p, me,
                       (CycleNode*)nullptr, (uint64_t)0, scal.p);
            const uint64_t ncl = d2h_scalar(c, scal.p);
            SBuf<CycleNode> cyc_local(c, ncl), cyc_all;
            W2R_CUDA(cudaMemsetAsync(scal.p, 0, 8, c.stream));
            W2R_LAUNCH(c, k_collect_cycle_nodes, grid(nn, 256), 256, 0, st, (const uint32_t*)next0.p, (const RankState*)cur, (const uint32_t*)lpiece, piece0, (const RankState*)S.p, me,
                       cyc_local.p, ncl, scal.p);
            std::vector<uint64_t> coff;
            allgather_v(cyc_local.p, ncl, cyc_all, coff);
            std::vector<CycleNode> cn(coff[W]);
            W2R_CUDA(cudaMemcpyAsync(cn.data(), cyc_all.p, cn.size() * sizeof(CycleNode), cudaMemcpyDeviceToHost, c.stream));
            W2R_CUDA(cudaStreamSynchronize(c.stream));
            std::vector<uint32_t> lab(np, NIL);
            for (uint64_t i = 0; i < np; ++i) {
                if ((S_h[i].y & RANK_RESOLVED) || lab[i] != NIL) continue;
                uint32_t mn = (uint32_t)i;
                for (uint32_t j = nxt_h[i]; j != i; j = nxt_h[j]) mn = std::min(mn, j);
                lab[i] = mn;
                for (uint32_t j = nxt_h[i]; j != i; j = nxt_h[j]) lab[j] = mn;
            }
            std::sort(cn.begin(), cn.end(), [&](const CycleNode& a, const CycleNode& b) {
                const uint32_t la = lab[a.piece], lb = lab[b.piece];
                if (la != lb) return la < lb;
                if (a.w0 != b.w0) return a.w0 < b.w0;
                if (a.w1 != b.w1) return a.w1 < b.w1;
                return a.gid < b.gid;
            });
            std::vector<uint64_t> heads_g, tails_g;
            for (size_t i = 0; i < cn.size(); ++i) {
                if (i > 0 && lab[cn[i].piece] == lab[cn[i - 1].piece]) continue;
                for (size_t j = i; j < cn.size() && lab[cn[j].piece] == lab[cn[i].piece] && cn[j].w0 == cn[i].w0 && cn[j].w1 == cn[i].w1; ++j)
                    if (cn[j].gid & 1ull) tails_g.push_back(cn[j].gid); else heads_g.push_back(cn[j].gid);
            }
            std::sort(heads_g.begin(), heads_g.end()); std::sort(tails_g.begin(), tails_g.end());
            SBuf<uint64_t> hg(c, heads_g.size() + 1), tg(c, tails_g.size() + 1);
            W2R_CUDA(cudaMemcpyAsync(hg.p, heads_g.data(), heads_g.size() * 8, cudaMemcpyHostToDevice, c.stream));
            W2R_CUDA(cudaMemcpyAsync(tg.p, tails_g.data(), tails_g.size() * 8, cudaMemcpyHostToDevice, c.stream));
            if (ncl) W2R_LAUNCH(c, k_apply_cycle_cuts, grid(ncl, 256), 256, 0, st, next0.p, ghead.p, me, (const CycleNode*)cyc_local.p, ncl, (const uint64_t*)hg.p, (uint32_t)heads_g.size(),
                                (const uint64_t*)tg.p, (uint32_t)tails_g.size());
            W2R_CUDA(cudaStreamSynchronize(c.stream));
        }
        trace_mark("graph: pieces ranked");
        kt_.begin(W2RAP_KT_SG_EDGES);
        PieceView pv{pieces.p, flip.p, S.p, np};
        SBuf<uint8_t> is_head(c, np + 4), keepp(c, np + 4);
        SBuf<uint32_t> chain_n(c, np + 1);
        is_head.zero(); keepp.zero();
        if (np) W2R_LAUNCH(c, k_chain_tails, grid(np, 256), 256, 0, pv, (const uint32_t*)nxt.p, is_head.p, chain_n.p, keepp.p, flags.p + 2);
        SBuf<PieceInfo> pinfo(c, np + 1);
        if (np) W2R_LAUNCH(c, k_piece_info, grid(np, 256), 256, 0, pv, pinfo.p);
        if (npl_last) W2R_LAUNCH(c, k_piece_keep_odd, grid(npl_last, 256), 256, 0, st, (const uint32_t*)next0.p, (const PieceRec*)pieces.p, (const PieceInfo*)pinfo.p, piece0, npl_last, keepp.p);
        xt.start();
        if (np) nccl_check(NcclApi::get().AllReduce(keepp.p, keepp.p, np, ncclUint8, ncclMax, comm, c.stream), "all-reduce");
        xms += xt.stop();
        if (d2h_scalar(c, flags.p + 2)) W2R_FAIL(W2RAP_ERR_EDGE_TOO_LONG, "an edge is longer than 2^24 k-mers (reference: KDef offset is 24 bits)");
        trace_mark("graph: strands");
        SBuf<uint32_t> h_piece(c, np + 1), h_n(c, np + 1);
        SBuf<uint64_t> h_w0(c, np + 1), h_w1(c, np + 1);
        W2R_CUDA(cudaMemsetAsync(scal.p, 0, 8, c.stream));
        if (np) W2R_LAUNCH(c, k_collect_head_pieces, grid(np, 256), 256, 0, pv, (const uint8_t*)is_head.p, (const uint8_t*)keepp.p, (const uint32_t*)chain_n.p, h_piece.p, h_w0.p, h_w1.p, h_n.p, scal.p, np);
        E = d2h_scalar(c, scal.p);
        SBuf<uint32_t> edge_of_piece(c, np + 1); edge_of_piece.fill_ff();
        edges_from_heads(h_piece, h_n, h_w0, h_w1, edge_of_piece);
        if (np) W2R_LAUNCH(c, k_piece_edges, grid(np, 256), 256, 0, pinfo.p, np, (const uint32_t*)edge_of_piece.p);
        kt_.end();
        W2R_TIMED(W2RAP_KT_EMIT_EDGES, W2R_LAUNCH(c, k_emit_edges_sharded, grid(nn, 256), 256, 0, st, (const uint32_t*)next0.p, (const RankState*)cur, (const uint32_t*)lpiece,
                                                   (const PieceInfo*)pinfo.p + piece0, (const uint64_t*)edge_off.p, edge_bases.p));
        kt_.begin(W2RAP_KT_SG_EDGES);
        xt.start();
        const uint64_t ebw = (edge_bytes + 3) / 4;
        if (ebw) nccl_check(NcclApi::get().AllReduce(edge_bases.p, edge_bases.p, ebw, ncclUint32, ncclSum, comm, c.stream), "all-reduce");
        xchg_bytes += ebw * 4 + np;
        kt_.end();
        kt_.begin(W2RAP_KT_SG_DICT);
        trace_mark("graph: edges");
        xms += xt.stop();
        next0.release(); ghead.release(); A.release(); B.release();
        pieces.release(); nxt.release(); flip.release(); S.release();
        uint64_t ecap = std::max<uint64_t>(1024, n_local / W + n_local / (4 * W));
        SBuf<SolidSlot> ebuck;
        SBuf<unsigned long long> ecount(c, W);
        std::vector<unsigned long long> en(W, 0);
        for (int attempt = 0;; ++attempt) {
            if (attempt > 2) W2R_FAIL(W2RAP_ERR_INTERNAL, "dictionary slice buffers did not converge");
            ebuck.alloc(c, W * ecap);
            ecount.zero();
            W2R_LAUNCH(c, k_dump_owned_sliced, grid(st.size(), 256), 256, 0, st, W, ebuck.p, ecap, ecount.p);
            W2R_CUDA(cudaMemcpyAsync(en.data(), ecount.p, W * 8, cudaMemcpyDeviceToHost, c.stream));
            W2R_CUDA(cudaStreamSynchronize(c.stream));
            unsigned long long mx = 0, sum = 0;
            for (auto v : en) { mx = std::max(mx, v); sum += v; }
            if (sum != n_local) W2R_FAIL(W2RAP_ERR_INTERNAL, "owned entries lost in the local table");
            if (mx <= ecap) break;
            ecap = mx + mx / 64 + 64;
        }
        solid_slots.release();
        xt.start();
        SBuf<unsigned long long> ercount(c, W);
        alltoall_slabs(ecount.p, ercount.p, sizeof(unsigned long long));
        std::vector<unsigned long long> ern(W, 0);
        W2R_CUDA(cudaMemcpyAsync(ern.data(), ercount.p, W * 8, cudaMemcpyDeviceToHost, c.stream));
        W2R_CUDA(cudaStreamSynchronize(c.stream));
        std::vector<size_t> es_off(W), es_cnt(W), er_off(W), er_cnt(W);
// ... 123 lines not shown
        SBuf<PathMeta> meta2(c, n_ovf);
        if (n_ovf) {
            W2R_CUDA(cudaMemsetAsync(counters.p + 3, 0, 8, c.stream));
            W2R_LAUNCH(c, k_collect_overflow, grid(n, 256), 256, 0, meta.p, n, olist.p, counters.p + 3);
            W2R_TIMED(W2RAP_KT_PATH_READS, launch_path(grid(n_ovf, block, path_occ_grid), olist.p, n_ovf, stage2.p, cap2, left2, row_off2.p, meta2.p));
            W2R_CUDA(cudaMemsetAsync(counters.p + 2, 0, 8, c.stream));
            W2R_LAUNCH(c, k_path_lens, grid(n_ovf, 256), 256, 0, meta2.p, (const uint32_t*)olist.p, n_ovf, lens.p, counters.p);
            W2R_CUDA(cudaMemcpyAsync(cnt, counters.p, 24, cudaMemcpyDeviceToHost, c.stream));
            W2R_CUDA(cudaStreamSynchronize(c.stream));
            if (cnt[2]) W2R_FAIL(W2RAP_ERR_INTERNAL, "a read path overflowed the worst-case staging row");
        }
        *pathed = cnt[0]; *multipathed = cnt[1];
        SBuf<unsigned long long> tot(c, 1);
        exclusive_scan<uint32_t, unsigned long long>(c, lens.p, n, (unsigned long long*)d_path_off.p, tot.p);
        *n_path_edges = d2h_scalar(c, tot.p);
        W2R_CUDA(cudaMemcpyAsync(d_path_off.p + n, n_path_edges, 8, cudaMemcpyHostToDevice, c.stream));
        W2R_CUDA(cudaStreamSynchronize(c.stream));
        d_path_edges.alloc(c, *n_path_edges);
        W2R_LAUNCH(c, k_path_gather, grid(n, 256), 256, 0, stage.p, cap, meta.p, (const uint32_t*)nullptr, row_off.p, d_path_off.p, n, d_path_edges.p, d_offset.p);
        if (n_ovf) W2R_LAUNCH(c, k_path_gather, grid(n_ovf, 256), 256, 0, stage2.p, cap2, meta2.p, (const uint32_t*)olist.p, row_off2.p, d_path_off.p, n_ovf, d_path_edges.p, d_offset.p);
        W2R_CUDA(cudaStreamSynchronize(c.stream));
    }

    struct PlaceSet { SBuf<uint64_t> off; SBuf<int32_t> edges; uint64_t n = 0, n_edges = 0; };
    void unique_places(PlaceSet& in, PlaceSet& res, bool sorted) {
        const uint64_t M = in.n;
        res.n = res.n_edges = 0;
        if (M == 0) { res.off.alloc(c, 1); res.off.zero(); res.edges.alloc(c, 1); return; }
        if (M >= (1ull << 32) - 8) W2R_FAIL(W2RAP_ERR_OOM, "more than 2^32 places");
        PlacesView s{in.off.p, in.edges.p, M};
        SBuf<uint64_t> h(c, M);
        SBuf<uint32_t> perm(c, M), tmp(c, M), first(c, M), excl(c, M), tot(c, 1);
        SBuf<unsigned long long> coll(c, 1);
        for (int attempt = 0;; ++attempt) {
            W2R_LAUNCH(c, k_place_hash, grid(M, 256), 256, 0, s, 0x1234567ull + 0x9e3779b97f4a7c15ull * (uint64_t)attempt, h.p);
            W2R_LAUNCH(c, k_rs_iota, grid(M, 256), 256, 0, perm.p, (uint32_t)M);
            SortWord w{h.p, 0, 64};
            radix_sort_perm(c, perm.p, tmp.p, (uint32_t)M, &w, 1);
            coll.zero();
            W2R_LAUNCH(c, k_place_first, grid(M, 256), 256, 0, s, (const uint32_t*)perm.p, (const uint64_t*)h.p, first.p, coll.p);
            if (!d2h_scalar(c, coll.p)) break;
            if (attempt == 3) W2R_FAIL(W2RAP_ERR_INTERNAL, "place hashes collide under four salts");
        }
        exclusive_scan<uint32_t, uint32_t>(c, first.p, M, excl.p, tot.p);
        const uint64_t U = d2h_scalar(c, tot.p);
        SBuf<uint32_t> rep(c, U), order;
        SBuf<unsigned int> maxlen(c, 1); maxlen.zero();
        W2R_LAUNCH(c, k_place_select, grid(M, 256), 256, 0, s, (const uint32_t*)perm.p, (const uint32_t*)first.p, (const uint32_t*)excl.p, rep.p, maxlen.p);
        if (sorted && U > 1) {
            const uint32_t ml = d2h_scalar(c, maxlen.p);
            order.alloc(c, U);
            SBuf<uint32_t> tmp2(c, U);
            SBuf<uint64_t> key(c, U);
            W2R_LAUNCH(c, k_rs_iota, grid(U, 256), 256, 0, order.p, (uint32_t)U);
            int bits = 1;
            while ((1ull << bits) < nh + 2) ++bits;
            for (uint32_t pos = ml; pos-- > 0;) {
                W2R_LAUNCH(c, k_place_key, grid(U, 256), 256, 0, s, (const uint32_t*)rep.p, U, pos, key.p);
                SortWord w{key.p, 0, bits};
                radix_sort_perm(c, order.p, tmp2.p, (uint32_t)U, &w, 1);
            }
        }
        SBuf<uint32_t> olen(c, U);
        SBuf<uint64_t> tote(c, 1);
        W2R_LAUNCH(c, k_place_out_len, grid(U, 256), 256, 0, s, (const uint32_t*)rep.p, (const uint32_t*)order.p, U, olen.p);
        res.off.alloc(c, U + 1);
        exclusive_scan<uint32_t, uint64_t>(c, olen.p, U, res.off.p, tote.p);
        W2R_CUDA(cudaMemcpyAsync(res.off.p + U, tote.p, 8, cudaMemcpyDeviceToDevice, c.stream));
        const uint64_t ne = d2h_scalar(c, tote.p);
        res.edges.alloc(c, ne + 1);
        W2R_LAUNCH(c, k_place_gather, grid(U, 256), 256, 0, s, (const uint32_t*)rep.p, (const uint32_t*)order.p, U, (const uint64_t*)res.off.p, res.edges.p);
        res.n = U; res.n_edges = ne;
    }
    void places_stage(SBuf<uint64_t>& d_path_off, SBuf<int32_t>& d_path_edges) {
        const uint64_t n = dr.n;
        PlaceSet local, uniq;
        {
            PathsView pv{d_path_off.p, d_path_edges.p, n};
            SBuf<uint32_t> plen(c, n + 1), kept(c, n + 1), pidx(c, n + 1), totk(c, 1);
            SBuf<uint8_t> flip(c, n + 1);
            SBuf<uint64_t> poff(c, n + 1), tote(c, 1);
            if (n) W2R_LAUNCH(c, k_place_measure, grid(n, 256), 256, 0, pv, (const uint32_t*)hcanon.p, (const uint32_t*)edge_len.p, (const int32_t*)involution.p, prm.places_K2, plen.p, kept.p, flip.p);
            exclusive_scan<uint32_t, uint32_t>(c, kept.p, n, pidx.p, totk.p);
            exclusive_scan<uint32_t, uint64_t>(c, plen.p, n, poff.p, tote.p);
            local.n = d2h_scalar(c, totk.p);
            local.n_edges = d2h_scalar(c, tote.p);
            local.off.alloc(c, local.n + 1); local.edges.alloc(c, local.n_edges + 1);
            if (n) W2R_LAUNCH(c, k_place_fill, grid(n, 256), 256, 0, pv, (const int32_t*)involution.p, (const uint32_t*)plen.p, (const uint8_t*)flip.p, (const uint32_t*)pidx.p,
                              (const uint64_t*)poff.p, local.off.p, local.edges.p);
            W2R_CUDA(cudaMemcpyAsync(local.off.p + local.n, tote.p, 8, cudaMemcpyDeviceToDevice, c.stream));
        }
        std::vector<unsigned long long> kt = {local.n};
        allreduce_u64(kt, ncclSum);
        out->n_places_kept = kt[0];
        if (world == 1) {
            unique_places(local, uniq, true);
        } else {
            PlaceSet mine, merged;
            unique_places(local, mine, false);
            local.off.release(); local.edges.release();
            SBuf<uint32_t> mylen(c, mine.n + 1), all_len;
            SBuf<uint64_t> tot(c, 1);
            if (mine.n) W2R_LAUNCH(c, k_place_lens, grid(mine.n, 256), 256, 0, (const uint64_t*)mine.off.p, mine.n, mylen.p);
            std::vector<uint64_t> loff, eoff;
            allgather_v(mylen.p, mine.n, all_len, loff);
            allgather_v(mine.edges.p, mine.n_edges, merged.edges, eoff);
            merged.n = loff[world]; merged.n_edges = eoff[world];
            merged.off.alloc(c, merged.n + 1);
            exclusive_scan<uint32_t, uint64_t>(c, all_len.p, merged.n, merged.off.p, tot.p);
            W2R_CUDA(cudaMemcpyAsync(merged.off.p + merged.n, tot.p, 8, cudaMemcpyDeviceToDevice, c.stream));
            unique_places(merged, uniq, true);
        }
        out->n_places = uniq.n; out->n_place_edges = uniq.n_edges;
        if (!(world > 1 && prm.graph_on_root_only && rank != 0)) {
            out->place_off = to_host<uint64_t>(uniq.off.p, uniq.n + 1);
            out->place_edges = to_host<int32_t>(uniq.edges.p, uniq.n_edges);
        }
        W2R_CUDA(cudaStreamSynchronize(c.stream));
    }

    template <class T>
    T* to_host(const T* dptr, size_t n, cudaStream_t s = nullptr) {
        T* h = out_alloc<T>(owner, n);
        if (!n) return h;
        if (s && ((uintptr_t)h & 15) == 0 && ((uintptr_t)dptr & 15) == 0) {
            k_copy_to_host<<<32, 512, 0, s>>>((const uint8_t*)dptr, (uint8_t*)h, n * sizeof(T));
            W2R_CUDA(cudaGetLastError());
            c.launches++;
        } else {
            W2R_CUDA(cudaMemcpyAsync(h, dptr, n * sizeof(T), cudaMemcpyDeviceToHost, s ? s : c.stream));
        }
        return h;
    }
    cudaStream_t copy_stream = nullptr;

    void run() {
        W2R_CUDA(cudaStreamCreateWithFlags(&c.stream, cudaStreamNonBlocking));
        g_alloc_host_ms = 0;
        kt_.s = c.stream;
        c.verbose = prm.verbose != 0;
        StageTimer total(c), st_t(c);
        total.start();
        out->n_reads = dr.n; out->n_bases = dr.n_bases;
        say(c, "creating kmers from reads...");
        st_t.start(); count_stage();
        out->timings.count_ms = st_t.stop();
        good.release();
        if (world > 1) {
            say(c, "updating adjacencies, finding edges (unique paths): dictionary sharded over %d GPUs", world);
            st_t.start(); graph_stage_sharded(cs_solid, n_solid_local_, count_logP_); out->timings.unipath_ms = st_t.stop();
        } else {
            say(c, "updating adjacencies");
            st_t.start();
            W2R_TIMED(W2RAP_KT_ADJACENCY, W2R_LAUNCH(c, k_adjacency, grid(st.size(), 256), 256, 0, st));
            out->timings.adjacency_ms = st_t.stop();
            say(c, "finding edges (unique paths)");
            st_t.start(); unipath_stage(); out->timings.unipath_ms = st_t.stop();
        }
        say(c, "building graph...");
        st_t.start(); hbv_stage(); out->timings.hbv_ms = st_t.stop();
        out->n_edges = E; out->n_vertices = nv; out->n_hbv_edges = nh;
        W2R_CUDA(cudaStreamCreateWithFlags(&copy_stream, cudaStreamNonBlocking));
        out->edge_len = to_host<uint32_t>(edge_len.p, E, copy_stream);
        if (!(world > 1 && prm.graph_on_root_only && rank != 0)) {
            out->edge_off = to_host<uint64_t>(edge_off.p, E + 1, copy_stream);
            out->edge_bases = to_host<uint8_t>(edge_bases.p, edge_bytes, copy_stream);
            out->edge_vertices = to_host<int32_t>(edge_vertices.p, 4 * E, copy_stream);
            out->fwd_xlat = to_host<int32_t>(fwd_xlat.p, E, copy_stream);
            out->rev_xlat = to_host<int32_t>(rev_xlat.p, E, copy_stream);
            out->involution = to_host<int32_t>(involution.p, nh, copy_stream);
        }
        SBuf<int32_t> d_offset, d_path_edges; SBuf<uint64_t> d_path_off;
        uint64_t npe = 0; unsigned long long pathed = 0, multi = 0;
        if (prm.want_paths) {
            say(c, "pathing reads into graph...");
            st_t.start(); path_stage(d_offset, d_path_off, d_path_edges, &npe, &pathed, &multi); out->timings.path_ms = st_t.stop();
            say(c, "%llu / %llu reads pathed, %llu spanning junctions", pathed, (unsigned long long)dr.n, multi);
        }
        if (prm.places_K2) {
            say(c, "constructing places from %llu paths", (unsigned long long)dr.n);
            st_t.start(); places_stage(d_path_off, d_path_edges); out->timings.places_ms = st_t.stop();
            say(c, "sorting %llu places", (unsigned long long)out->n_places_kept);
            say(c, "%llu unique places", (unsigned long long)out->n_places);
        }
        st_t.start();
        SBuf<unsigned long long> dig(c, 2); dig.zero();
        {
            struct Part { const void* p; size_t bytes; } parts[] = {{edge_len.p, E * 4}, {edge_bases.p, edge_bytes}, {edge_vertices.p, 4 * E * 4}, {fwd_xlat.p, E * 4}, {rev_xlat.p, E * 4}};
            uint64_t salt = 1;
            for (const Part& pt : parts) { if (pt.bytes) W2R_LAUNCH(c, k_digest_words, grid((pt.bytes + 3) / 4, 256, 4), 256, 0, (const uint8_t*)pt.p, pt.bytes, salt << 40, dig.p); ++salt; }
            if (prm.want_paths && dr.n) W2R_LAUNCH(c, k_digest_paths, grid(dr.n, 256, 8), 256, 0, dr.view(), d_offset.p, d_path_off.p, d_path_edges.p, dig.p + 1);
        }
        unsigned long long dig_h[2] = {0, 0};
        W2R_CUDA(cudaMemcpyAsync(dig_h, dig.p, 16, cudaMemcpyDeviceToHost, c.stream));
        if (prm.want_paths) {
            out->n_paths = dr.n; out->n_path_edges = npe; out->n_pathed = pathed; out->n_multipathed = multi;
            out->path_offset = to_host<int32_t>(d_offset.p, dr.n);
            out->path_off = to_host<uint64_t>(d_path_off.p, dr.n + 1);
            out->path_edges = to_host<int32_t>(d_path_edges.p, npe);
        }
        wait_for_dictionary();
        if (prm.dump_kmers == 1 && out->n_solid) {
            const uint64_t n_mine = world > 1 ? n_slice_entries : out->n_solid;
            SBuf<DumpRec> dd(c, n_mine + 1), dd_all;
            SBuf<unsigned long long> cur(c, 1); cur.zero();
            W2R_LAUNCH(c, k_dump_solid, grid(st.size(), 256), 256, 0, st, dd.p, cur.p);
            const DumpRec* src = dd.p;
            if (world > 1) { std::vector<uint64_t> doff; allgather_v(dd.p, n_mine, dd_all, doff); src = dd_all.p; }
            dump_host.resize(out->n_solid);
            W2R_CUDA(cudaMemcpyAsync(dump_host.data(), src, out->n_solid * sizeof(DumpRec), cudaMemcpyDeviceToHost, c.stream));
            W2R_CUDA(cudaStreamSynchronize(c.stream));
        }
        W2R_CUDA(cudaStreamSynchronize(c.stream));
        W2R_CUDA(cudaStreamSynchronize(copy_stream));
        out->timings.d2h_ms = st_t.stop();
        if (E == 0 && out->edge_off) out->edge_off[0] = 0;
        uint64_t neb = 0;
        for (uint64_t i = 0; i < E; ++i) neb += out->edge_len[i];
        out->n_edge_bases = neb;
        if (prm.dump_kmers && !dump_host.empty()) {
            std::sort(dump_host.begin(), dump_host.end(), [](const DumpRec& a, const DumpRec& b) { return a.w0 < b.w0 || (a.w0 == b.w0 && a.w1 < b.w1); });
            out->n_dump = dump_host.size();
            out->dump = out_alloc<w2rap_kmer_rec>(owner, dump_host.size());
            static_assert(sizeof(DumpRec) == sizeof(w2rap_kmer_rec), "dump record layout");
            memcpy(out->dump, dump_host.data(), dump_host.size() * sizeof(DumpRec));
        }
        {
            uint64_t hd = 0;
            for (int i = 0; i <= 100; ++i) { uint64_t x = out->hist[i] + 0x9e3779b97f4a7c15ull * (uint64_t)(i + 1); x ^= x >> 33; x *= 0xff51afd7ed558ccdull; x ^= x >> 33; hd += x; }
            out->digest_graph = dig_h[0] + hd;
            std::vector<unsigned long long> dp = {dig_h[1]};
            allreduce_u64(dp, ncclSum);
            out->digest_paths = dp[0];
        }
        out->timings.total_ms = total.stop();
        kt_.resolve(out->timings.kernel_ms);
        out->timings.alloc_host_ms = (float)g_alloc_host_ms;
        out->timings.exchange_bytes = xchg_bytes;
        out->timings.count_exchange_bytes = xchg_count_bytes;
        out->timings.n_records = n_records;
        out->timings.kernel_launches = c.launches;
        out->timings.count_launches = c.count_launches;
        say(c, "%llu edges of total length %llu; %llu vertices", (unsigned long long)E, (unsigned long long)neb, (unsigned long long)nv);
    }

    ~Pipeline() {
        if (dict_stream) cudaStreamSynchronize(dict_stream);
        if (copy_stream) { cudaStreamSynchronize(copy_stream); cudaStreamDestroy(copy_stream); }
        good.release(); solid_slots.release(); edge_bases.release(); edge_off.release(); edge_len.release();
        edge_vertices.release(); fwd_xlat.release(); rev_xlat.release(); involution.release(); hleft.release();
        cs_scal.release(); cs_flags.release(); cs_hist.release(); cs_region.release(); cs_dump.release(); cs_solid.release();
        path_slices.release(); path_bloom.release(); hright.release(); from_e.release(); to_e.release();
        hcanon.release(); from_n.release(); to_n.release();
        if (dict_stream) { cudaStreamSynchronize(dict_stream); cudaStreamDestroy(dict_stream); cudaEventDestroy(dict_ready); }
        if (c.stream) { cudaStreamSynchronize(c.stream); cudaStreamDestroy(c.stream); }
    }
};

static void validate_reads(const w2rap_reads* in) {
    if (!in) W2R_FAIL(W2RAP_ERR_BAD_ARG, "null read store");
    if (in->n_reads && (!in->bases || !in->base_off || !in->len || !in->quals || !in->qual_off)) W2R_FAIL(W2RAP_ERR_BAD_ARG, "null pointer in read store");
    if (in->n_reads >= (1ull << 32)) W2R_FAIL(W2RAP_ERR_BAD_ARG, "more than 2^32-1 reads on one device");
}

struct UploadArena {
    std::mutex mu;
    bool in_use = false;
    void* buf[5] = {nullptr, nullptr, nullptr, nullptr, nullptr};
    size_t cap[5] = {0, 0, 0, 0, 0};
    static UploadArena& get(int device) { static UploadArena* a = new UploadArena[16]; return a[device & 15]; }
};
void arena_release(int device) { UploadArena& a = UploadArena::get(device); std::lock_guard<std::mutex> g(a.mu); a.in_use = false; }
static void dev_alloc(DeviceReads* d, void** p, size_t bytes, cudaStream_t s, int which) {
    if (d->arena) {
        UploadArena& a = UploadArena::get(d->device);
        if (a.cap[which] < bytes) {
            if (a.buf[which]) cudaFree(a.buf[which]);
            a.buf[which] = nullptr; a.cap[which] = 0;
            size_t want = bytes + bytes / 16;
            W2R_CUDA(cudaMalloc(&a.buf[which], want));
            a.cap[which] = want;
        }
        *p = a.buf[which];
        return;
    }
    if (d->pooled) W2R_CUDA(cudaMallocAsync(p, bytes, s)); else W2R_CUDA(cudaMalloc(p, bytes));
}
static int upload_batches_override() {
    static const int n = [] {
        const char* v = getenv("W2RAP_UPLOAD_BATCHES");
        if (!v) return 0;
        char* end = nullptr;
        const long x = strtol(v, &end, 10);
        return (end != v && *end == '\0' && x >= 1 && x <= (long)SMEM_MAX_BATCH) ? (int)x : -1;
    }();
    return n;
}

static void upload(const w2rap_reads* in, int device, DeviceReads* d, cudaStream_t s, bool batched) {
    const int forced_batches = batched ? upload_batches_override() : 0;
    if (forced_batches < 0) W2R_FAIL(W2RAP_ERR_BAD_ARG, "W2RAP_UPLOAD_BATCHES must be an integer in 1..%u (the most record runs per partition the count handles)", SMEM_MAX_BATCH);
    d->device = device;
    d->n = in->n_reads;
    const uint64_t n = d->n;
    d->bases_bytes = n ? in->base_off[n] : 0;
    d->quals_bytes = n ? in->qual_off[n] : 0;
    const double t0 = now_ms();
    {
        const unsigned nt = n > (1u << 20) ? 8u : 1u;
        std::vector<uint64_t> t_nb(nt, 0), t_inst(nt, 0), t_bad(nt, ~0ull), t_kr(nt, 0);
        std::vector<uint32_t> t_mx(nt, 0), t_kind(nt, 0);
        auto work = [&](unsigned t) {
            uint64_t lo = n * t / nt, hi = n * (t + 1) / nt, nb = 0, inst = 0, kr = 0; uint32_t mx = 0;
            for (uint64_t i = lo; i < hi; ++i) {
                uint32_t L = in->len[i];
                nb += L; if (L > mx) mx = L;
                if (L > 59) { inst += L - 59; ++kr; }
                if (in->base_off[i + 1] < in->base_off[i] || in->base_off[i + 1] - in->base_off[i] < (uint64_t)(L + 3) / 4) { t_bad[t] = i; t_kind[t] = 1; break; }
                if (in->qual_off[i + 1] <= in->qual_off[i]) { t_bad[t] = i; t_kind[t] = 2; break; }
            }
            t_nb[t] = nb; t_inst[t] = inst; t_mx[t] = mx; t_kr[t] = kr;
        };
        std::vector<std::thread> th;
        for (unsigned t = 1; t < nt; ++t) th.emplace_back(work, t);
        work(0);
        for (auto& x : th) x.join();
        uint64_t nb = 0, inst = 0, kr = 0; uint32_t mx = 0;
        for (unsigned t = 0; t < nt; ++t) {
            kr += t_kr[t];
            if (t_kind[t] == 1) W2R_FAIL(W2RAP_ERR_BAD_ARG, "read %llu: base offsets do not hold its bases", (unsigned long long)t_bad[t]);
            if (t_kind[t] == 2) W2R_FAIL(W2RAP_ERR_BAD_ARG, "read %llu: empty quality stream (at least the terminator byte is required)", (unsigned long long)t_bad[t]);
            nb += t_nb[t]; inst += t_inst[t]; mx = std::max(mx, t_mx[t]);
        }
        if (mx > 65535u) W2R_FAIL(W2RAP_ERR_BAD_ARG, "reads longer than 65535 bases are not supported (the reference stores good lengths in uint16_t)");
        d->n_bases = nb; d->max_len = mx; d->n_inst_upper = inst; d->n_kreads = kr;
    }
    const double t1 = now_ms();
    if (d->pooled) {
        UploadArena& a = UploadArena::get(device);
        std::lock_guard<std::mutex> g(a.mu);
        if (!a.in_use) { a.in_use = true; d->arena = true; }
    }
    dev_alloc(d, (void**)&d->bases, d->bases_bytes + 32, s, 0);
    dev_alloc(d, (void**)&d->quals, d->quals_bytes + 32, s, 1);
    dev_alloc(d, (void**)&d->base_off, (n + 1) * 8, s, 2);
    dev_alloc(d, (void**)&d->qual_off, (n + 1) * 8, s, 3);
    dev_alloc(d, (void**)&d->len, (n + 1) * 4, s, 4);
    W2R_CUDA(cudaMemsetAsync(d->bases + d->bases_bytes, 0, 32, s));
    W2R_CUDA(cudaMemsetAsync(d->quals + d->quals_bytes, 0, 32, s));
    const double t2 = now_ms();
    if (n) {
        const unsigned nbatch = forced_batches ? (unsigned)forced_batches : (batched && n >= (1u << 20)) ? 8u : 1u;
        for (unsigned b = 0; b < nbatch; ++b) {
            const uint64_t r0 = n * b / nbatch, r1 = n * (b + 1) / nbatch;
            const uint64_t b0 = in->base_off[r0], b1 = in->base_off[r1], q0 = in->qual_off[r0], q1 = in->qual_off[r1];
            W2R_CUDA(cudaMemcpyAsync(d->len + r0, in->len + r0, (r1 - r0) * 4, cudaMemcpyHostToDevice, s));
            W2R_CUDA(cudaMemcpyAsync(d->base_off + r0, in->base_off + r0, (r1 - r0 + 1) * 8, cudaMemcpyHostToDevice, s));
            W2R_CUDA(cudaMemcpyAsync(d->qual_off + r0, in->qual_off + r0, (r1 - r0 + 1) * 8, cudaMemcpyHostToDevice, s));
            W2R_CUDA(cudaMemcpyAsync(d->bases + b0, in->bases + b0, b1 - b0, cudaMemcpyHostToDevice, s));
            W2R_CUDA(cudaMemcpyAsync(d->quals + q0, in->quals + q0, q1 - q0, cudaMemcpyHostToDevice, s));
            if (batched) {
                cudaEvent_t e;
                W2R_CUDA(cudaEventCreateWithFlags(&e, cudaEventDisableTiming));
                W2R_CUDA(cudaEventRecord(e, s));
                d->batch_ready.push_back(e);
                d->batch_first.push_back(r0);
            }
        }
        if (batched) d->batch_first.push_back(n);
    } else {
        uint64_t z = 0;
        W2R_CUDA(cudaMemcpyAsync(d->base_off, &z, 8, cudaMemcpyHostToDevice, s));
        W2R_CUDA(cudaMemcpyAsync(d->qual_off, &z, 8, cudaMemcpyHostToDevice, s));
    }
    if (!batched) W2R_CUDA(cudaStreamSynchronize(s));
    if (getenv("W2RAP_TRACE")) fprintf(stderr, "[w2rap] upload: validate %.1f ms, alloc %.1f ms, enqueue %.1f ms\n", t1 - t0, t2 - t1, now_ms() - t2);
}

static void check_params(const w2rap_params* p) {
    if (!p) W2R_FAIL(W2RAP_ERR_BAD_ARG, "null params");
    if (p->abi_version != W2RAP_STEP2_ABI_VERSION) W2R_FAIL(W2RAP_ERR_BAD_ARG, "ABI version %u, library has %d", p->abi_version, W2RAP_STEP2_ABI_VERSION);
    if (p->K != W2RAP_K) W2R_FAIL(W2RAP_ERR_BAD_ARG, "K=%u: only K=60 is built (the reference hard-wires it, BuildReadQGraph.cc:51)", p->K);
    if (p->min_freq == 0 || p->min_freq > 255) W2R_FAIL(W2RAP_ERR_BAD_ARG, "min_freq must be in 1..255 (counts saturate at 255)");
    if (p->force_passes > 4096) W2R_FAIL(W2RAP_ERR_BAD_ARG, "force_passes must be <= 4096");
    if (p->places_K2 && (p->places_K2 < W2RAP_K || !p->want_paths || !p->apply_fixpaths))
        W2R_FAIL(W2RAP_ERR_BAD_ARG, "places_K2 needs want_paths and apply_fixpaths (step 3 reads the paths after FixPaths) and K2 >= 60");
}

}

struct w2rap_comm { int world, rank, device; w2r::ncclComm_t comm; };

namespace w2r {
static void run_on_device(DeviceReads& dr, const w2rap_params* p, w2rap_graph* out, float h2d_ms, const w2rap_comm* cm = nullptr, double t_entry = 0) {
    GraphOwner* owner = new GraphOwner();
    memset(out, 0, sizeof(*out));
    out->_owner = owner;
    try {
        { Ctx probe; check_device(dr.device, probe); }
        SlabLease lease(dr.device);
        Pipeline pl(dr, *p, out, owner);
        if (cm) { pl.world = cm->world; pl.rank = cm->rank; pl.comm = cm->comm; }
// ... 183 lines not shown
```

### w2rap-contigger_b200/csrc/unipath.cuh

```cuda
#pragma once
#include "kmer.cuh"

namespace w2r {

constexpr uint32_t RANK_RESOLVED = 0x80000000u;
constexpr uint32_t EMPTY_NODE = 0xfffffffeu;
constexpr uint32_t GHOST_TAIL = 0xfffffffdu;
W2R_HD bool slot_is_ghost(const SolidSlot& s) { return s.pad != 0; }

W2R_HD Kmer node_kmer(const SolidTable& t, uint32_t x) {
    const SolidSlot& s = t.slots[x >> 1];
    Kmer k{s.w0, s.w1};
    return (x & 1u) ? kmer_rc(k) : k;
}

W2R_HD uint32_t unipath_succ_link(const SolidTable& t, uint32_t x, int* missing, bool* to_ghost = nullptr) {
    const SolidSlot& s = t.slots[x >> 1];
    if (to_ghost) *to_ghost = false;
    if (s.w0 == EMPTY_W0) return EMPTY_NODE;
    if (slot_is_ghost(s)) return GHOST_TAIL;
    Kmer k{s.w0, s.w1};
    Kmer rc = kmer_rc(k);
    if (rc == k) return NIL;
    const bool o = x & 1u;
    Kmer xk = o ? rc : k;
    uint32_t c = o ? ctx_rc(s.ctx & 0xffu) : (s.ctx & 0xffu);
    if (nib_count(c) != 1) return NIL;
    Kmer n = kmer_succ(xk, nib_single(c));
    Kmer nrc = kmer_rc(n);
    if (nrc == n) return NIL;
    bool rev = kmer_less(nrc, n);
    int64_t ts = solid_find(t, rev ? nrc : n);
    if (ts < 0) { if (missing) *missing = 1; return NIL; }
    uint32_t c2 = t.slots[ts].ctx & 0xffu;
    if (rev) c2 = ctx_rc(c2);
    if (nib_count(c2 >> 4) != 1) return NIL;
    if (to_ghost) *to_ghost = slot_is_ghost(t.slots[ts]);
    return (uint32_t)(2 * ts) + (rev ? 1u : 0u);
}

W2R_HD uint32_t pruned_context(const SolidTable& t, Kmer k, uint32_t c) {
    for (uint32_t b = 0; b < 4; ++b)
        if (c & (1u << b)) { if (solid_find_any(t, kmer_succ(k, b), nullptr) < 0) c &= ~(1u << b); }
    for (uint32_t b = 0; b < 4; ++b)
        if (c & (16u << b)) { if (solid_find_any(t, kmer_pred(k, b), nullptr) < 0) c &= ~(16u << b); }
    return c;
}


struct alignas(8) RankState { uint32_t x, y; };

W2R_HD RankState rank_init_node(const uint32_t* next0, uint32_t x) {
    uint32_t nx = next0[x];
    return nx >= GHOST_TAIL ? RankState{x, RANK_RESOLVED} : RankState{nx, 1u};
}

constexpr uint32_t SPLITTER_MASK = 63u;
W2R_HD bool hash_splitter(uint32_t x) { uint32_t h = x * 0x9e3779b1u; h ^= h >> 15; h *= 0x85ebca77u; h ^= h >> 13; return (h & SPLITTER_MASK) == 0; }
W2R_HD bool node_is_splitter(const uint32_t* next0, const uint8_t* ghead, uint32_t x) {
    const uint32_t nx = next0[x];
    if (nx == EMPTY_NODE || nx == GHOST_TAIL) return false;
    return next0[x ^ 1u] == NIL || (ghead && ghead[x]) || hash_splitter(x);
}
W2R_HD void splitter_walk(const uint32_t* next0, uint32_t s, RankState* label, RankState* S) {
    uint32_t y = s, o = 0, ny = next0[s];
    for (;;) {
        label[y] = RankState{s, o};
        if (ny == NIL) { S[s] = RankState{y, o | RANK_RESOLVED}; return; }
        const uint32_t nny = next0[ny];
        if (nny == GHOST_TAIL) { S[s] = RankState{y, o | RANK_RESOLVED}; return; }
        ++o;
        if (hash_splitter(ny) || ny == s) { S[s] = RankState{ny, o}; return; }
        y = ny; ny = nny;
    }
}
W2R_HD RankState splitter_finish_node(const uint32_t* next0, const RankState* label, const RankState* S, uint32_t y) {
    if (next0[y] == EMPTY_NODE || next0[y] == GHOST_TAIL) return RankState{y, RANK_RESOLVED};
    RankState l = label[y];
    if (l.x == NIL) return RankState{y, 0};
    RankState st = S[l.x];
    if (!(st.y & RANK_RESOLVED)) return RankState{y, 0};
    return RankState{st.x, ((st.y & ~RANK_RESOLVED) - l.y) | RANK_RESOLVED};
}
W2R_HD RankState rank_step_node(const RankState* A, uint32_t x, bool* unresolved) {
    RankState a = A[x];
    *unresolved = false;
    if (!(a.y & RANK_RESOLVED)) {
        RankState b = A[a.x];
        a = RankState{b.x, (a.y + (b.y & ~RANK_RESOLVED)) | (b.y & RANK_RESOLVED)};
        *unresolved = !(a.y & RANK_RESOLVED);
    }
    return a;
}
W2R_HD RankState cycle_step_node(const SolidTable& t, const RankState* A, uint32_t x, bool* changed) {
    RankState a = A[x], b = A[a.x];
    uint32_t best = a.y;
    if (b.y != a.y) {
        const SolidSlot& sa = t.slots[a.y]; const SolidSlot& sb = t.slots[b.y];
        if (kmer_less(Kmer{sb.w0, sb.w1}, Kmer{sa.w0, sa.w1})) best = b.y;
    }
    *changed = best != a.y;
    return RankState{b.x, best};
}
W2R_HD void cycle_cut_node(const RankState* A, uint32_t* next0, uint32_t x) {
    if ((x & 1u) == 0 && A[x].y == (x >> 1)) {
        uint32_t y = next0[x ^ 1u];
        next0[y ^ 1u] = NIL;
        next0[x ^ 1u] = NIL;
    }
}
W2R_HD bool strand_decide_node(const SolidTable& t, const RankState* R, uint32_t x, uint8_t* keep) {
    if (t.slots[x >> 1].w0 == EMPTY_W0) return false;
    RankState a = R[x], f = R[x ^ 1u];
    uint32_t d = a.y & ~RANK_RESOLVED, off = f.y & ~RANK_RESOLVED;
    uint64_t n = (uint64_t)d + off + 1;
    uint32_t head = f.x ^ 1u;
    uint64_t L = n + K - 1;
    if (L & 1) {
        uint64_t m = L / 2, ostar = m < n - 1 ? m : n - 1;
        if (off == ostar) keep[head] = (kmer_base(node_kmer(t, x), (int)(m - off)) & 2u) ? 0 : 1;
    } else if (off == 0) {
        Kmer hk = node_kmer(t, x);
        Kmer ok = node_kmer(t, a.x ^ 1u);
        keep[x] = (kmer_less(hk, ok) || (hk == ok && (x & 1u) == 0)) ? 1 : 0;
    }
    return off == 0 && n > 0x1000000ull;
}
W2R_HD bool head_is_kept(const SolidTable& t, const RankState* R, const uint8_t* keep, uint32_t x) {
    return t.slots[x >> 1].w0 != EMPTY_W0 && (R[x ^ 1u].y & ~RANK_RESOLVED) == 0 && keep[x];
}
template <class Put>
W2R_HD void emit_node(const SolidTable& t, const RankState* R, const uint32_t* edge_of_head, const uint64_t* edge_off, uint32_t x, Put& put) {
    SolidSlot* s = t.slots + (x >> 1);
    if (s->w0 == EMPTY_W0) return;
    RankState f = R[x ^ 1u];
    uint32_t e = edge_of_head[f.x ^ 1u];
    if (e == NIL) return;
    uint32_t off = f.y & ~RANK_RESOLVED;
    s->edge = e; s->off = off;
    Kmer k = node_kmer(t, x);
    uint64_t bo = edge_off[e];
    put(bo, (uint64_t)off, kmer_first(k));
    if ((R[x].y & ~RANK_RESOLVED) == 0)
        for (int i = 1; i < K; ++i) put(bo, (uint64_t)off + i, kmer_base(k, i));
}

struct EndKey { uint64_t h, k0, k1; };
W2R_HD bool edge_end_key(const uint8_t* p, uint32_t len, uint32_t w, bool* is_pal, EndKey* out) {
    bool pal = false;
    if (len == (uint32_t)K) {
        uint64_t w0 = 0, w1 = 0;
        for (int i = 0; i < 32; ++i) w0 = (w0 << 2) | packed_base(p, i);
        for (int i = 32; i < K; ++i) w1 = (w1 << 2) | packed_base(p, i);
        pal = kmer_is_palindrome(Kmer{w0, w1 << 8});
    }
    *is_pal = pal;
    if (pal && w >= 2) { *out = EndKey{~0ull, ~0ull, ~0ull}; return false; }
    bool rc = w >= 2, distal = w & 1u;
    uint64_t start = distal ? len - (K - 1) : 0;
    uint64_t h = 14695981039346656037ull, a = 0, b = 0;
    for (int i = 0; i < K - 1; ++i) {
        uint64_t pos = start + i;
        uint32_t c = rc ? 3u - packed_base(p, len - 1 - pos) : packed_base(p, pos);
        h = 1099511628211ull * (h ^ (uint64_t)c);
        if (i < 32) a = (a << 2) | c; else b = (b << 2) | c;
    }
    *out = EndKey{h, a, b << 10};
    return true;
}

}
```

Before: 26.77.

## Run unipath stage on dense minimizer-sorted solid node array instead of hash table

Each partition's solid k-mers are compacted in shared memory, bitonic-sorted by minimizer hash and offset, and then written out contiguously, so neighbouring k-mers land near each other. A dense SolidSlot array is built during insertion, with the hash table storing the dense index. The adjacency, links, list ranking, strand decision, head collection and edge emission then iterate over the n_solid dense nodes instead of all hash slots, and results are backfilled into the table afterwards. The aim is to cut wasted work on empty slots and improve locality of neighbour lookups, at the cost of an extra dense buffer, an indirection in node_find, a per-partition sort and a backfill pass.

```diff
diff --git a/w2rap-contigger_b200/csrc/count_part.cuh b/w2rap-contigger_b200/csrc/count_part.cuh
--- a/w2rap-contigger_b200/csrc/count_part.cuh
+++ b/w2rap-contigger_b200/csrc/count_part.cuh
@@ -266,6 +266,8 @@
     __shared__ unsigned int sh_hist[104];
     __shared__ int sh_fail;
     __shared__ uint32_t sh_tot[2], sh_cnt[2];
+    __shared__ uint32_t sh_nsolid;
+    __shared__ unsigned long long sh_solid_base;
     const uint32_t lane = threadIdx.x & 31u, warp = threadIdx.x >> 5, nwarp = blockDim.x >> 5;
     const unsigned le_mask = (2u << lane) - 1u;
     for (int j = threadIdx.x; j < 104; j += blockDim.x) sh_hist[j] = 0;
@@ -314,7 +316,7 @@
             uint4* cw = reinterpret_cast<uint4*>(ccs);
             for (uint32_t j = threadIdx.x; j < SMEM_SLOTS / 4; j += blockDim.x) cw[j] = make_uint4(0, 0, 0, 0);
         }
-        if (threadIdx.x == 0) sh_fail = 0;
+        if (threadIdx.x == 0) { sh_fail = 0; sh_nsolid = 0; }
         __syncthreads();
         auto insert = [&](const Kmer k, const uint32_t ctx) {
             uint32_t s = smem_slot_hash(k) >> (32 - sp.log_slots);
@@ -394,13 +396,70 @@
                 const unsigned ones = __ballot_sync(0xffffffffu, occ && c == 1u);
                 if (lane == 0 && ones) atomicAdd(&sh_hist[1], (unsigned)__popc(ones));
                 if (occ && c != 1u) atomicAdd(&sh_hist[c > 100u ? 100u : c], 1u);
-                const bool solid = occ && c >= sp.min_freq;
-                const uint64_t pos = warp_append(sp.solid_cursor, solid);
-                if (solid) { if (pos < sp.solid_cap) sp.solid_out[pos] = make_ulonglong2(kk.x, kk.y | ctx); else atomicExch(sp.solid_overflow, 1); }
+                if (occ) keys[j] = c >= sp.min_freq ? make_ulonglong2(kk.x, kk.y | ctx) : make_ulonglong2(~0ull, ~0ull);
                 if (sp.dump_out) {
                     const uint64_t dp = warp_append(sp.dump_cursor, occ);
                     if (occ) sp.dump_out[dp] = DumpRec{kk.x, kk.y, c, ctx, NIL, 0};
                 }
+            }
+            __syncthreads();
+            for (uint32_t base = 0; base < SMEM_SLOTS; base += blockDim.x) {
+                const uint32_t j = base + threadIdx.x;
+                const bool solid = j < SMEM_SLOTS && keys[j].x != ~0ull;
+                const unsigned m = __ballot_sync(0xffffffffu, solid);
+                uint32_t first = 0;
+                if (lane == 0 && m) first = atomicAdd(&sh_nsolid, (uint32_t)__popc(m));
+                first = __shfl_sync(0xffffffffu, first, 0);
+                if (solid) ccs[first + __popc(m & (le_mask >> 1))] = j;
+            }
+            __syncthreads();
+            const uint32_t ns = sh_nsolid, N = ns <= 1u ? ns : 1u << (32 - __clz(ns - 1u));
+            for (uint32_t i = threadIdx.x; i < ns; i += blockDim.x) {
+                const uint32_t j = ccs[i];
+                const ulonglong2 kk = keys[j];
+                uint32_t off;
+                const uint32_t mh = kmer_minimizer_offset_words(Kmer{kk.x, kk.y & ~0xffull}, &off);
+                ccs[i] = (mh & 0x1fffu) << 19 | off << 13 | j;
+            }
+            if (N <= blockDim.x) {
+                const uint32_t i = threadIdx.x;
+                __syncthreads();
+                uint32_t v = i < ns ? ccs[i] : ~0u;
+                for (uint32_t kb = 2; kb <= N; kb <<= 1) {
+                    for (uint32_t jb = kb >> 1; jb > 0; jb >>= 1) {
+                        uint32_t o;
+                        if (jb >= 32u) {
+                            __syncthreads();
+                            if (i < N) ccs[i] = v;
+                            __syncthreads();
+                            o = i < N ? ccs[i ^ jb] : ~0u;
+                        } else o = __shfl_xor_sync(0xffffffffu, v, jb);
+                        const bool keep_min = ((i & jb) == 0) == ((i & kb) == 0);
+                        v = keep_min ? (v < o ? v : o) : (v < o ? o : v);
+                    }
+                }
+                __syncthreads();
+                if (i < N) ccs[i] = v;
+            } else {
+                for (uint32_t i = ns + threadIdx.x; i < N; i += blockDim.x) ccs[i] = ~0u;
+                __syncthreads();
+                for (uint32_t kb = 2; kb <= N; kb <<= 1) {
+                    for (uint32_t jb = kb >> 1; jb > 0; jb >>= 1) {
+                        if (jb > 32u) __syncthreads();
+                        for (uint32_t t = threadIdx.x; t < N / 2; t += blockDim.x) {
+                            const uint32_t i = 2 * t - (t & (jb - 1u));
+                            const uint32_t a = ccs[i], b = ccs[i + jb];
+                            if ((a > b) == ((i & kb) == 0)) { ccs[i] = b; ccs[i + jb] = a; }
+                        }
+                        if (jb > 32u) __syncthreads(); else __syncwarp();
+                    }
+                }
+            }
+            if (threadIdx.x == 0 && ns) sh_solid_base = atomicAdd(sp.solid_cursor, (unsigned long long)ns);
+            __syncthreads();
+            for (uint32_t i = threadIdx.x; i < ns; i += blockDim.x) {
+                const uint64_t pos = sh_solid_base + i;
+                if (pos < sp.solid_cap) sp.solid_out[pos] = keys[ccs[i] & 0x1fffu]; else atomicExch(sp.solid_overflow, 1);
             }
         }
         __syncthreads();
diff --git a/w2rap-contigger_b200/csrc/extract.cuh b/w2rap-contigger_b200/csrc/extract.cuh
--- a/w2rap-contigger_b200/csrc/extract.cuh
+++ b/w2rap-contigger_b200/csrc/extract.cuh
@@ -78,11 +78,11 @@
 
 constexpr int MINI_M = 15;
 constexpr int MINI_W = K - MINI_M + 1;
+W2R_HD uint32_t mmer_rc(uint32_t v) { return rev2_32(~v) >> (32 - 2 * MINI_M); }
+W2R_HD uint32_t mmer_mix(uint32_t c) { c ^= c >> 16; c *= 0x85ebca6bu; c ^= c >> 13; c *= 0xc2b2ae35u; c ^= c >> 16; return c; }
 W2R_HD uint32_t mmer_hash_of(uint32_t v) {
-    const uint32_t rc = rev2_32(~v) >> (32 - 2 * MINI_M);
-    uint32_t c = v < rc ? v : rc;
-    c ^= c >> 16; c *= 0x85ebca6bu; c ^= c >> 13; c *= 0xc2b2ae35u; c ^= c >> 16;
-    return c;
+    const uint32_t rc = mmer_rc(v);
+    return mmer_mix(v < rc ? v : rc);
 }
 W2R_HD uint32_t mmer_hash_at(const uint8_t* bases, uint64_t pos) { return mmer_hash_of(bases16_at(bases, pos) & ((1u << (2 * MINI_M)) - 1u)); }
 W2R_HD uint32_t mini_mix(uint32_t wmin) {
@@ -102,6 +102,25 @@
     }
     return m;
 }
+W2R_HD uint32_t mmer_bits_at(uint64_t lo, uint64_t hi, int bit) {
+    const uint64_t w = bit == 0 ? lo : (bit < 64 ? (lo >> bit) | (hi << (64 - bit)) : hi >> (bit - 64));
+    return (uint32_t)w & ((1u << (2 * MINI_M)) - 1u);
+}
+W2R_HD uint32_t kmer_minimizer_offset_words(Kmer k, uint32_t* offset) {
+    const uint64_t lo = rev2(k.w0), hi = rev2(k.w1);
+    const uint64_t rlo = (~k.w1 >> 8) | (~k.w0 << 56), rhi = ~k.w0 >> 8;
+    uint32_t m = 0xffffffffu, off = 0;
+#if defined(__CUDA_ARCH__)
+#pragma unroll
+#endif
+    for (int t = 0; t < MINI_W; ++t) {
+        const uint32_t v = mmer_bits_at(lo, hi, 2 * t), rc = mmer_bits_at(rlo, rhi, 2 * (MINI_W - 1 - t));
+        const uint32_t h = mmer_mix(v < rc ? v : rc), o = v < rc ? (uint32_t)t : (uint32_t)(MINI_W - 1 - t);
+        if (h < m || (h == m && o < off)) { m = h; off = o; }
+    }
+    *offset = off;
+    return m;
+}
 W2R_HD uint32_t kmer_minimizer_hash(const uint8_t* bases, uint64_t j) {
     uint32_t m = 0xffffffffu;
     for (int t = 0; t < MINI_W; ++t) { const uint32_t h = mmer_hash_at(bases, j + t); if (h < m) m = h; }
diff --git a/w2rap-contigger_b200/csrc/kernels.cuh b/w2rap-contigger_b200/csrc/kernels.cuh
--- a/w2rap-contigger_b200/csrc/kernels.cuh
+++ b/w2rap-contigger_b200/csrc/kernels.cuh
@@ -89,7 +89,8 @@
     }
 }
 
-__global__ void k_insert_solid(const ulonglong2* __restrict__ recs, uint64_t n, SolidTable st, uint32_t* __restrict__ bloom, uint32_t bloom_W, uint32_t slice_words) {
+__global__ void k_insert_solid(const ulonglong2* __restrict__ recs, uint64_t n, SolidTable st, uint32_t* __restrict__ bloom, uint32_t bloom_W, uint32_t slice_words,
+                               SolidSlot* __restrict__ dense) {
     for (uint64_t i = (uint64_t)blockIdx.x * blockDim.x + threadIdx.x; i < n; i += (uint64_t)gridDim.x * blockDim.x) {
         ulonglong2 rec = __ldcs(recs + i);
         Kmer k{rec.x, rec.y & ~0xffull};
@@ -99,9 +100,10 @@
         for (;;) {
             SolidSlot* p = st.slots + h;
             U128 old = cas128(p, ~0ull, ~0ull, k.w0, k.w1);
-            if (old.lo == ~0ull && old.hi == ~0ull) { p->ctx = ctx; p->edge = NIL; p->off = 0; p->pad = 0; break; }
+            if (old.lo == ~0ull && old.hi == ~0ull) { p->ctx = ctx; p->edge = NIL; p->off = dense ? (uint32_t)i : 0u; p->pad = 0; break; }
             h = st.next(h);
         }
+        if (dense) dense[i] = SolidSlot{k.w0, k.w1, ctx, NIL, 0, 0};
     }
 }
 __global__ void k_insert_entries(const SolidSlot* __restrict__ recs, uint64_t n, SolidTable st, uint32_t* __restrict__ bloom, uint32_t bloom_W, uint32_t slice_words) {
@@ -128,8 +130,16 @@
         if (c2 != c) s->ctx = c2;
     }
 }
-
-__global__ void k_links(SolidTable st, uint32_t* __restrict__ next0, int* __restrict__ missing) {
+__global__ void k_adjacency_dense(DenseNodes d) {
+    for (uint64_t i = (uint64_t)blockIdx.x * blockDim.x + threadIdx.x; i < d.n; i += (uint64_t)gridDim.x * blockDim.x) {
+        SolidSlot* s = d.nodes + i;
+        const uint32_t c = s->ctx & 0xffu, c2 = pruned_context(d.t, Kmer{s->w0, s->w1}, c);
+        if (c2 != c) s->ctx = c2;
+    }
+}
+
+template <class V>
+__global__ void k_links(V st, uint32_t* __restrict__ next0, int* __restrict__ missing) {
     const uint64_t nn = 2 * st.size();
     for (uint64_t x = (uint64_t)blockIdx.x * blockDim.x + threadIdx.x; x < nn; x += (uint64_t)gridDim.x * blockDim.x) {
         int miss = 0;
@@ -221,7 +231,8 @@
         A[x] = RankState{next0[x], x >> 1};
     }
 }
-__global__ void k_cycle_step(const uint32_t* __restrict__ list, uint64_t n, SolidTable st, const RankState* __restrict__ A, RankState* __restrict__ B, int* __restrict__ changed) {
+template <class V>
+__global__ void k_cycle_step(const uint32_t* __restrict__ list, uint64_t n, V st, const RankState* __restrict__ A, RankState* __restrict__ B, int* __restrict__ changed) {
     for (uint64_t i = (uint64_t)blockIdx.x * blockDim.x + threadIdx.x; i < n; i += (uint64_t)gridDim.x * blockDim.x) {
         uint32_t x = list[i];
         bool ch;
@@ -234,13 +245,15 @@
         cycle_cut_node(A, next0, list[i]);
     }
 }
-__global__ void k_strand_decide(SolidTable st, const RankState* __restrict__ R, uint8_t* __restrict__ keep, int* __restrict__ too_long) {
+template <class V>
+__global__ void k_strand_decide(V st, const RankState* __restrict__ R, uint8_t* __restrict__ keep, int* __restrict__ too_long) {
     const uint64_t nn = 2 * st.size();
     for (uint64_t xi = (uint64_t)blockIdx.x * blockDim.x + threadIdx.x; xi < nn; xi += (uint64_t)gridDim.x * blockDim.x) {
         if (strand_decide_node(st, R, (uint32_t)xi, keep)) atomicExch(too_long, 1);
     }
 }
-__global__ void k_collect_heads(SolidTable st, const RankState* __restrict__ R, const uint8_t* __restrict__ keep, uint32_t* __restrict__ h_node,
+template <class V>
+__global__ void k_collect_heads(V st, const RankState* __restrict__ R, const uint8_t* __restrict__ keep, uint32_t* __restrict__ h_node,
                                 uint64_t* __restrict__ h_w0, uint64_t* __restrict__ h_w1, uint32_t* __restrict__ h_n, unsigned long long* cursor, uint64_t cap) {
     const uint64_t nn = 2 * st.size();
     for (uint64_t base = (uint64_t)blockIdx.x * blockDim.x; base < nn; base += (uint64_t)gridDim.x * blockDim.x) {
@@ -272,11 +285,21 @@
         atomicOr(reinterpret_cast<uint32_t*>(bases + (addr & ~3ull)), b << (8 * (uint32_t)(addr & 3ull) + 2 * (uint32_t)(pos & 3ull)));
     }
 };
-__global__ void k_emit_edges(SolidTable st, const RankState* __restrict__ R, const uint32_t* __restrict__ edge_of_head, const uint64_t* __restrict__ edge_off,
+template <class V>
+__global__ void k_emit_edges(V st, const RankState* __restrict__ R, const uint32_t* __restrict__ edge_of_head, const uint64_t* __restrict__ edge_off,
                              uint8_t* __restrict__ edge_bases) {
     const uint64_t nn = 2 * st.size();
     OrBase put{edge_bases};
     for (uint64_t xi = (uint64_t)blockIdx.x * blockDim.x + threadIdx.x; xi < nn; xi += (uint64_t)gridDim.x * blockDim.x) emit_node(st, R, edge_of_head, edge_off, (uint32_t)xi, put);
+}
+__global__ void k_backfill_slots(SolidTable st, const SolidSlot* __restrict__ dense) {
+    const uint64_t T = st.size();
+    for (uint64_t i = (uint64_t)blockIdx.x * blockDim.x + threadIdx.x; i < T; i += (uint64_t)gridDim.x * blockDim.x) {
+        SolidSlot* s = st.slots + i;
+        if (s->w0 == EMPTY_W0) continue;
+        const SolidSlot& d = dense[s->off];
+        s->ctx = d.ctx; s->edge = d.edge; s->off = d.off;
+    }
 }
 
 __global__ void k_copy_to_host(const uint8_t* __restrict__ src, uint8_t* __restrict__ dst, size_t bytes) {
diff --git a/w2rap-contigger_b200/csrc/pipeline.cu b/w2rap-contigger_b200/csrc/pipeline.cu
--- a/w2rap-contigger_b200/csrc/pipeline.cu
+++ b/w2rap-contigger_b200/csrc/pipeline.cu
@@ -307,6 +307,8 @@
     SBuf<uint16_t> good;
     SBuf<SolidSlot> solid_slots;
     SolidTable st{nullptr, 0};
+    SBuf<SolidSlot> dense_slots;
+    DenseNodes dn{{nullptr, 0}, nullptr, 0};
     uint64_t E = 0, nv = 0, nh = 0;
     SBuf<uint8_t> edge_bases; SBuf<uint64_t> edge_off; SBuf<uint32_t> edge_len;
     SBuf<int32_t> edge_vertices, fwd_xlat, rev_xlat, involution, hleft, hright, from_e, to_e;
@@ -782,19 +784,22 @@
         if (world > 1) return;
         EventTimer kt(c.stream);
         kt.start();
+        if (n_solid > (1ull << 31) - 8) W2R_FAIL(W2RAP_ERR_OOM, "too many solid k-mers for one device's graph stage (32-bit oriented node ids); shard over more GPUs");
         const uint64_t nslots = solid_table_slots(n_solid);
-        if (nslots > (1ull << 31) - 8) W2R_FAIL(W2RAP_ERR_OOM, "too many solid k-mers for one device's graph stage (32-bit oriented node ids); shard over more GPUs");
         solid_slots.alloc(c, nslots);
         solid_slots.fill_ff();
         st = SolidTable{solid_slots.p, nslots};
+        dense_slots.alloc(c, n_solid);
+        dn = DenseNodes{st, dense_slots.p, n_solid};
         alloc_path_filter(n_solid);
         if (n_solid) W2R_TIMED(W2RAP_KT_INSERT_SOLID, W2R_LAUNCH(c, k_insert_solid, grid(n_solid, 256), 256, 0, (const ulonglong2*)cs_solid.p, n_solid, st,
-                                                                   path_slice_words ? path_bloom.p : nullptr, 1u, path_slice_words));
+                                                                   path_slice_words ? path_bloom.p : nullptr, 1u, path_slice_words, dense_slots.p));
         out->timings.dict_ms = kt.stop();
         cs_solid.release();
     }
 
-    void list_ranking(SBuf<uint32_t>& next0, const uint8_t* ghead, uint64_t nn, SBuf<RankState>& A, SBuf<RankState>& B, RankState** cur_out, RankState** oth_out) {
+    template <class V>
+    void list_ranking(const V& nodes, SBuf<uint32_t>& next0, const uint8_t* ghead, uint64_t nn, SBuf<RankState>& A, SBuf<RankState>& B, RankState** cur_out, RankState** oth_out) {
         SBuf<int> flags(c, 4); flags.zero();
         SBuf<unsigned long long> scal(c, 4); scal.zero();
         W2R_LAUNCH(c, k_count_splitters, grid(nn, 256), 256, 0, next0.p, ghead, nn, scal.p + 3);
@@ -830,7 +835,7 @@
             W2R_LAUNCH(c, k_cycle_init, grid(ncyc, 256), 256, 0, list.p, ncyc, next0.p, x0);
             for (int round = 0; round < 40; ++round) {
                 W2R_CUDA(cudaMemsetAsync(flags.p + 1, 0, sizeof(int), c.stream));
-                W2R_LAUNCH(c, k_cycle_step, grid(ncyc, 256), 256, 0, list.p, ncyc, st, x0, x1, flags.p + 1);
+                W2R_LAUNCH(c, k_cycle_step, grid(ncyc, 256), 256, 0, list.p, ncyc, nodes, x0, x1, flags.p + 1);
                 std::swap(x0, x1);
                 if (!d2h_scalar(c, flags.p + 1)) break;
             }
@@ -871,29 +876,31 @@
     }
 
     void unipath_stage() {
-        const uint64_t T = st.size(), nn = 2 * T;
+        const uint64_t nn = 2 * dn.size();
         SBuf<uint32_t> next0(c, nn);
         SBuf<int> flags(c, 4); flags.zero();
         SBuf<unsigned long long> scal(c, 4); scal.zero();
-        W2R_TIMED(W2RAP_KT_LINKS, W2R_LAUNCH(c, k_links, grid(nn, 256), 256, 0, st, next0.p, flags.p));
+        W2R_TIMED(W2RAP_KT_LINKS, W2R_LAUNCH(c, k_links, grid(nn, 256), 256, 0, dn, next0.p, flags.p));
         if (d2h_scalar(c, flags.p)) W2R_FAIL(W2RAP_ERR_INTERNAL, "a neighbour k-mer promised by a pruned context is missing (reference: ForceAssert in EdgeBuilder::lookup)");
-        SBuf<RankState> A(c, nn), B(c, nn);
+        SBuf<RankState> A(c, std::max<uint64_t>(nn, 1)), B(c, std::max<uint64_t>(nn, 1));
         RankState* cur = nullptr; RankState* oth = nullptr;
-        list_ranking(next0, nullptr, nn, A, B, &cur, &oth);
+        list_ranking(dn, next0, nullptr, nn, A, B, &cur, &oth);
         const RankState* R = cur;
         SBuf<uint8_t> keep(c, nn); keep.zero();
-        W2R_LAUNCH(c, k_strand_decide, grid(nn, 256), 256, 0, st, R, keep.p, flags.p + 2);
+        W2R_LAUNCH(c, k_strand_decide, grid(nn, 256), 256, 0, dn, R, keep.p, flags.p + 2);
         if (d2h_scalar(c, flags.p + 2)) W2R_FAIL(W2RAP_ERR_EDGE_TOO_LONG, "an edge is longer than 2^24 k-mers (reference: KDef offset is 24 bits)");
         uint64_t cap = out->n_solid;
         SBuf<uint32_t> h_node(c, cap), h_n(c, cap);
         SBuf<uint64_t> h_w0(c, cap), h_w1(c, cap);
         W2R_CUDA(cudaMemsetAsync(scal.p + 2, 0, 8, c.stream));
-        W2R_LAUNCH(c, k_collect_heads, grid(nn, 256), 256, 0, st, R, keep.p, h_node.p, h_w0.p, h_w1.p, h_n.p, scal.p + 2, cap);
+        W2R_LAUNCH(c, k_collect_heads, grid(nn, 256), 256, 0, dn, R, keep.p, h_node.p, h_w0.p, h_w1.p, h_n.p, scal.p + 2, cap);
         E = d2h_scalar(c, scal.p + 2);
         if (E > cap) W2R_FAIL(W2RAP_ERR_INTERNAL, "more edges than solid k-mers");
         SBuf<uint32_t> edge_of_head(c, nn); edge_of_head.fill_ff();
         edges_from_heads(h_node, h_n, h_w0, h_w1, edge_of_head);
-        W2R_TIMED(W2RAP_KT_EMIT_EDGES, W2R_LAUNCH(c, k_emit_edges, grid(nn, 256), 256, 0, st, R, edge_of_head.p, edge_off.p, edge_bases.p));
+        W2R_TIMED(W2RAP_KT_EMIT_EDGES, W2R_LAUNCH(c, k_emit_edges, grid(nn, 256), 256, 0, dn, R, edge_of_head.p, edge_off.p, edge_bases.p));
+        W2R_LAUNCH(c, k_backfill_slots, grid(st.size(), 256), 256, 0, st, (const SolidSlot*)dense_slots.p);
+        dense_slots.release(); dn = DenseNodes{st, nullptr, 0};
         W2R_CUDA(cudaStreamSynchronize(c.stream));
     }
 
@@ -950,7 +957,7 @@
         solid_slots.alloc(c, nslots);
         solid_slots.fill_ff();
         st = SolidTable{solid_slots.p, nslots};
-        if (n_local) W2R_TIMED(W2RAP_KT_INSERT_SOLID, W2R_LAUNCH(c, k_insert_solid, grid(n_local, 256), 256, 0, (const ulonglong2*)solid.p, n_local, st, (uint32_t*)nullptr, 1u, 0u));
+        if (n_local) W2R_TIMED(W2RAP_KT_INSERT_SOLID, W2R_LAUNCH(c, k_insert_solid, grid(n_local, 256), 256, 0, (const ulonglong2*)solid.p, n_local, st, (uint32_t*)nullptr, 1u, 0u, (SolidSlot*)nullptr));
         solid.release();
         trace_mark("graph: local table");
         kt_.begin(W2RAP_KT_SG_QUERIES);
@@ -1003,7 +1010,7 @@
         uint32_t* lpiece = nullptr;
         for (int iteration = 0;; ++iteration) {
             if (iteration > 1) W2R_FAIL(W2RAP_ERR_INTERNAL, "circles left after cutting them");
-            list_ranking(next0, ghead.p, nn, A, B, &cur, &oth);
+            list_ranking(st, next0, ghead.p, nn, A, B, &cur, &oth);
             trace_mark("graph: links+list ranking");
             kt_.begin(W2RAP_KT_SG_PIECES);
             lpiece = reinterpret_cast<uint32_t*>(oth);
@@ -1433,7 +1440,7 @@
         } else {
             say(c, "updating adjacencies");
             st_t.start();
-            W2R_TIMED(W2RAP_KT_ADJACENCY, W2R_LAUNCH(c, k_adjacency, grid(st.size(), 256), 256, 0, st));
+            W2R_TIMED(W2RAP_KT_ADJACENCY, W2R_LAUNCH(c, k_adjacency_dense, grid(dn.size(), 256), 256, 0, dn));
             out->timings.adjacency_ms = st_t.stop();
             say(c, "finding edges (unique paths)");
             st_t.start(); unipath_stage(); out->timings.unipath_ms = st_t.stop();
@@ -1528,7 +1535,7 @@
     ~Pipeline() {
         if (dict_stream) cudaStreamSynchronize(dict_stream);
         if (copy_stream) { cudaStreamSynchronize(copy_stream); cudaStreamDestroy(copy_stream); }
-        good.release(); solid_slots.release(); edge_bases.release(); edge_off.release(); edge_len.release();
+        good.release(); solid_slots.release(); dense_slots.release(); edge_bases.release(); edge_off.release(); edge_len.release();
         edge_vertices.release(); fwd_xlat.release(); rev_xlat.release(); involution.release(); hleft.release();
         cs_scal.release(); cs_flags.release(); cs_hist.release(); cs_region.release(); cs_dump.release(); cs_solid.release();
         path_slices.release(); path_bloom.release(); hright.release(); from_e.release(); to_e.release();
diff --git a/w2rap-contigger_b200/csrc/unipath.cuh b/w2rap-contigger_b200/csrc/unipath.cuh
--- a/w2rap-contigger_b200/csrc/unipath.cuh
+++ b/w2rap-contigger_b200/csrc/unipath.cuh
@@ -8,14 +8,30 @@
 constexpr uint32_t GHOST_TAIL = 0xfffffffdu;
 W2R_HD bool slot_is_ghost(const SolidSlot& s) { return s.pad != 0; }
 
-W2R_HD Kmer node_kmer(const SolidTable& t, uint32_t x) {
-    const SolidSlot& s = t.slots[x >> 1];
+struct DenseNodes {
+    SolidTable t;
+    SolidSlot* nodes;
+    uint64_t n;
+    W2R_HD uint64_t size() const { return n; }
+};
+W2R_HD SolidSlot& node_entry(const SolidTable& t, uint64_t id) { return t.slots[id]; }
+W2R_HD SolidSlot& node_entry(const DenseNodes& d, uint64_t id) { return d.nodes[id]; }
+W2R_HD int64_t node_find(const SolidTable& t, Kmer k) { return solid_find(t, k); }
+W2R_HD int64_t node_find(const DenseNodes& d, Kmer k) {
+    const int64_t s = solid_find(d.t, k);
+    return s < 0 ? -1 : (int64_t)d.t.slots[s].off;
+}
+
+template <class V>
+W2R_HD Kmer node_kmer(const V& v, uint32_t x) {
+    const SolidSlot& s = node_entry(v, x >> 1);
     Kmer k{s.w0, s.w1};
     return (x & 1u) ? kmer_rc(k) : k;
 }
 
-W2R_HD uint32_t unipath_succ_link(const SolidTable& t, uint32_t x, int* missing, bool* to_ghost = nullptr) {
-    const SolidSlot& s = t.slots[x >> 1];
+template <class V>
+W2R_HD uint32_t unipath_succ_link(const V& t, uint32_t x, int* missing, bool* to_ghost = nullptr) {
+    const SolidSlot& s = node_entry(t, x >> 1);
     if (to_ghost) *to_ghost = false;
     if (s.w0 == EMPTY_W0) return EMPTY_NODE;
     if (slot_is_ghost(s)) return GHOST_TAIL;
@@ -30,12 +46,12 @@
     Kmer nrc = kmer_rc(n);
     if (nrc == n) return NIL;
     bool rev = kmer_less(nrc, n);
-    int64_t ts = solid_find(t, rev ? nrc : n);
+    int64_t ts = node_find(t, rev ? nrc : n);
     if (ts < 0) { if (missing) *missing = 1; return NIL; }
-    uint32_t c2 = t.slots[ts].ctx & 0xffu;
+    uint32_t c2 = node_entry(t, ts).ctx & 0xffu;
     if (rev) c2 = ctx_rc(c2);
     if (nib_count(c2 >> 4) != 1) return NIL;
-    if (to_ghost) *to_ghost = slot_is_ghost(t.slots[ts]);
+    if (to_ghost) *to_ghost = slot_is_ghost(node_entry(t, ts));
     return (uint32_t)(2 * ts) + (rev ? 1u : 0u);
 }
 
@@ -92,11 +108,12 @@
     }
     return a;
 }
-W2R_HD RankState cycle_step_node(const SolidTable& t, const RankState* A, uint32_t x, bool* changed) {
+template <class V>
+W2R_HD RankState cycle_step_node(const V& t, const RankState* A, uint32_t x, bool* changed) {
     RankState a = A[x], b = A[a.x];
     uint32_t best = a.y;
     if (b.y != a.y) {
-        const SolidSlot& sa = t.slots[a.y]; const SolidSlot& sb = t.slots[b.y];
+        const SolidSlot& sa = node_entry(t, a.y); const SolidSlot& sb = node_entry(t, b.y);
         if (kmer_less(Kmer{sb.w0, sb.w1}, Kmer{sa.w0, sa.w1})) best = b.y;
     }
     *changed = best != a.y;
@@ -109,8 +126,9 @@
         next0[x ^ 1u] = NIL;
     }
 }
-W2R_HD bool strand_decide_node(const SolidTable& t, const RankState* R, uint32_t x, uint8_t* keep) {
-    if (t.slots[x >> 1].w0 == EMPTY_W0) return false;
+template <class V>
+W2R_HD bool strand_decide_node(const V& t, const RankState* R, uint32_t x, uint8_t* keep) {
+    if (node_entry(t, x >> 1).w0 == EMPTY_W0) return false;
     RankState a = R[x], f = R[x ^ 1u];
     uint32_t d = a.y & ~RANK_RESOLVED, off = f.y & ~RANK_RESOLVED;
     uint64_t n = (uint64_t)d + off + 1;
@@ -126,12 +144,13 @@
     }
     return off == 0 && n > 0x1000000ull;
 }
-W2R_HD bool head_is_kept(const SolidTable& t, const RankState* R, const uint8_t* keep, uint32_t x) {
-    return t.slots[x >> 1].w0 != EMPTY_W0 && (R[x ^ 1u].y & ~RANK_RESOLVED) == 0 && keep[x];
+template <class V>
+W2R_HD bool head_is_kept(const V& t, const RankState* R, const uint8_t* keep, uint32_t x) {
+    return node_entry(t, x >> 1).w0 != EMPTY_W0 && (R[x ^ 1u].y & ~RANK_RESOLVED) == 0 && keep[x];
 }
-template <class Put>
-W2R_HD void emit_node(const SolidTable& t, const RankState* R, const uint32_t* edge_of_head, const uint64_t* edge_off, uint32_t x, Put& put) {
-    SolidSlot* s = t.slots + (x >> 1);
+template <class V, class Put>
+W2R_HD void emit_node(const V& t, const RankState* R, const uint32_t* edge_of_head, const uint64_t* edge_off, uint32_t x, Put& put) {
+    SolidSlot* s = &node_entry(t, x >> 1);
     if (s->w0 == EMPTY_W0) return;
     RankState f = R[x ^ 1u];
     uint32_t e = edge_of_head[f.x ^ 1u];
```

Result: faster. 27.60 (median of 6 runs) (+3.1%).
